# bab2min/Kiwi

Hardware: AMD Instinct MI355X
Metric: sentences/sec on batched analyze(), device kernels with inputs resident in HBM (dictionary scan + lattice + Viterbi/Knlm, top-1); host-to-host rate: see e2e (higher is better)
Workload: dtype int32+f32; 1 GPU; c2-64k: 65536 synthetic sentences ({'exact_jamo': 40}), synthetic 'full' model (kiwi_amd/synth.py), Knlm, top-1; sentences_per_gpu=65536, chunks_per_gpu=65536, jamo_per_gpu=2621440, parallelism=shard1, device_bytes=9402884427, rerun_chunks=0

## Files before the change

### include/kiwi_amd.h

```cpp
#ifndef KIWI_AMD_H
#define KIWI_AMD_H
#include <stddef.h>
#include <stdint.h>
#ifdef __cplusplus
extern "C" {
#endif

typedef struct kamd_engine* kamd_engine_h;
typedef struct kamd_batch* kamd_batch_h;
typedef struct kamd_results* kamd_results_h;

typedef struct
{
	uint32_t position, word_position, sent_position, line_number;
	uint16_t length; uint8_t tag; uint8_t sense_or_script;
	float score, typo_cost;
	uint32_t typo_form_id, paired_token, sub_sent_position;
	uint16_t dialect; uint16_t form_len;
	int32_t morph_id;
	uint64_t form_off;
} kamd_token_t;

kamd_engine_h kamd_open(const char* raw_model_path, int device);
kamd_engine_h kamd_open_dialects(const char* raw_model_path, int device, int enabled_dialects);
kamd_engine_h kamd_open_mode(const char* raw_model_path, int device, int lm_mode, int enabled_dialects);
void kamd_close(kamd_engine_h h);
const char* kamd_last_error(void);

int kamd_set_config(kamd_engine_h h, float cut_off_threshold, float space_penalty, float typo_cost_weight,
	uint32_t max_unk_form_size, uint32_t max_unk_form_size_followed_by_jclass, uint32_t space_tolerance, int integrate_allomorph);
int kamd_set_oov_chr_bias(kamd_engine_h h, float bias);
int kamd_set_oov_freq_params(kamd_engine_h h, float global_weight, float local_weight, float global_min_freq);

kamd_results_h kamd_analyze_batch(kamd_engine_h h, const uint16_t* texts, const uint64_t* offsets, uint32_t n,
	uint32_t top_n, uint64_t match_options, int open_ending, int host_threads);

kamd_batch_h kamd_stage(kamd_engine_h h, const uint16_t* texts, const uint64_t* offsets, uint32_t n, uint64_t match_options, int open_ending, int host_threads);
int kamd_run(kamd_engine_h h, kamd_batch_h b, float* ms_out);
kamd_results_h kamd_fetch(kamd_engine_h h, kamd_batch_h b, uint32_t top_n);
int kamd_batch_info(kamd_batch_h b, uint64_t* info3);
int kamd_batch_reruns(kamd_batch_h b, float* ms_out);
int kamd_batch_pool(kamd_batch_h b, uint64_t* out3);
void kamd_batch_close(kamd_batch_h b);

uint32_t kamd_res_texts(kamd_results_h r);
uint32_t kamd_res_size(kamd_results_h r, uint32_t text);
float kamd_res_prob(kamd_results_h r, uint32_t text, uint32_t index);
uint32_t kamd_res_token_num(kamd_results_h r, uint32_t text, uint32_t index);
const kamd_token_t* kamd_res_tokens(kamd_results_h r, uint32_t text, uint32_t index);
const uint16_t* kamd_res_forms(kamd_results_h r, uint32_t text);
uint64_t kamd_res_d2h_bytes(kamd_results_h r);
void kamd_res_close(kamd_results_h r);
size_t kamd_res_pack(kamd_results_h r, uint8_t* out, size_t cap);
kamd_results_h kamd_res_merge_strided(const uint8_t* const* parts, const size_t* sizes, uint32_t n_parts);

int kamd_debug_exact_math(const float* x, float* exp_out, float* log_out, uint32_t n);
int kamd_debug_exact_tanh(const float* x, float* tanh_out, uint32_t n);
int kamd_debug_cong_global(kamd_engine_h h, const uint32_t* ctx, const uint32_t* hist7, const uint32_t* next, const uint8_t* flags, float* out, uint32_t n);
uint64_t kamd_debug_match_pattern(uint16_t left, const uint16_t* text, uint32_t len, uint64_t match_options);
int kamd_debug_sbg_next(const char* raw_model_path, uint32_t* hist8, uint32_t* pos, uint32_t wid, float knlm_ll, float* ll_out);
typedef struct kamd_typo* kamd_typo_h;
kamd_typo_h kamd_typo_new(float continual_cost, float lengthening_cost);
void kamd_typo_close(kamd_typo_h t);
kamd_typo_h kamd_typo_default(int default_typo_set);
int kamd_typo_add(kamd_typo_h t, const uint16_t* orig, uint32_t n_orig, const uint16_t* error, uint32_t n_error, float cost, int left_cond, int dialect);
int kamd_typo_add_entry(kamd_typo_h t, const uint16_t* orig, uint32_t n_orig, const uint16_t* error, uint32_t n_error, float cost, int left_cond, int dialect);
int kamd_typo_set_costs(kamd_typo_h t, float continual_cost, float lengthening_cost);
int kamd_typo_scale(kamd_typo_h t, float scale);
int kamd_typo_prepare(kamd_typo_h t, int inverse);
size_t kamd_typo_graph(kamd_typo_h t, const uint16_t* text, uint32_t len, int allowed_dialect, int normalize_coda, uint8_t* out, size_t cap);
kamd_results_h kamd_analyze_batch_typo(kamd_engine_h h, kamd_typo_h t, float threshold, int allowed_dialect, const uint16_t* texts, const uint64_t* offsets, uint32_t n_texts,
                                       uint32_t top_n, uint64_t match_options, int open_ending, int host_threads);
kamd_batch_h kamd_stage_typo(kamd_engine_h h, kamd_typo_h t, float threshold, int allowed_dialect, const uint16_t* texts, const uint64_t* offsets, uint32_t n_texts,
                             uint64_t match_options, int open_ending, int host_threads);
typedef struct kamd_morphset* kamd_morphset_h;
kamd_morphset_h kamd_morphset_new(kamd_engine_h h);
int kamd_morphset_add(kamd_morphset_h m, const uint16_t* form, uint32_t len, int tag);
void kamd_morphset_close(kamd_morphset_h m);
kamd_results_h kamd_analyze_batch_opt(kamd_engine_h h, kamd_typo_h t, float threshold, int allowed_dialect, kamd_morphset_h blocklist,
                                      const uint16_t* texts, const uint64_t* offsets, uint32_t n_texts, uint32_t top_n, uint64_t match_options, int open_ending, int host_threads);
kamd_results_h kamd_analyze_batch_dialect(kamd_engine_h h, kamd_typo_h t, float threshold, int allowed_dialect, float dialect_cost, kamd_morphset_h blocklist,
                                          const uint16_t* texts, const uint64_t* offsets, uint32_t n_texts, uint32_t top_n, uint64_t match_options, int open_ending, int host_threads);
kamd_results_h kamd_analyze_pretokenized(kamd_engine_h h, const uint16_t* text, uint32_t len, uint32_t top_n, uint64_t match_options, int open_ending,
                                         const uint32_t* spans, uint32_t n_spans, const uint16_t* forms);
size_t kamd_typo_graph_device(kamd_engine_h h, kamd_typo_h t, const uint16_t* text, uint32_t len, int allowed_dialect, int normalize_coda, int use_device, uint8_t* out, size_t cap);
size_t kamd_typo_lattices(kamd_engine_h h, kamd_typo_h t, float threshold, int allowed_dialect, const uint16_t* text, uint32_t len, uint64_t match_options, uint8_t* out, size_t cap);
size_t kamd_dump_dict(kamd_engine_h h, uint8_t* out, size_t cap);
size_t kamd_dump_lattices(kamd_engine_h h, const uint16_t* text, uint32_t len, uint64_t match_options, uint8_t* out, size_t cap);

int kamd_cong_info(kamd_engine_h h, uint32_t* vocab, uint32_t* contexts, uint32_t* dim);
int kamd_cong_topk(kamd_engine_h h, int kind, const uint32_t* ids, const uint32_t* bg_ids, const float* weights, uint32_t n, uint32_t top_n,
                   uint32_t* out_ids, float* out_scores, uint32_t* out_counts);
int kamd_cong_pairs(kamd_engine_h h, int kind, const uint32_t* a, const uint32_t* b, uint32_t n, float* out);
int kamd_cong_to_context_id(kamd_engine_h h, const uint32_t* ids, uint32_t n, uint32_t* out_context);
int64_t kamd_cong_from_context_id(kamd_engine_h h, uint32_t context_id, uint32_t* out, uint64_t max_size);
int kamd_cong_inv_norms(kamd_engine_h h, int contexts, float* out);
int64_t kamd_cong_table(kamd_engine_h h, int contexts, uint8_t* out, uint64_t cap);

#ifdef __cplusplus
}
#endif
#endif
```

### kiwi_amd/csrc/capi_low.cpp

```cpp
#include <cstddef>
#include <cstring>
#include <memory>
#include <mutex>
#include <string>
#include "../../include/kiwi_amd.h"
#include "engine.hpp"
#include "sbg_eval.hpp"
#include "typo.hpp"

using namespace kamd;

struct kamd_engine { std::unique_ptr<Engine> e; };
struct kamd_batch { std::shared_ptr<StagedBatch> b; };
struct kamd_results { BatchResults r; };
static_assert(sizeof(kamd_token_t) == sizeof(FlatToken) && offsetof(kamd_token_t, form_off) == offsetof(FlatToken, formOff) && offsetof(kamd_token_t, morph_id) == offsetof(FlatToken, morph),
	"kamd_token_t is the layout of kamd::FlatToken");

namespace kamd { void exactMathProbe(const float* x, float* e, float* l, float* t, uint32_t n); }
namespace kamd { void conggProbe(const FlatModel& m, const uint32_t* ctx, const uint32_t* hist, const uint32_t* next, const uint8_t* flags, float* out, uint32_t n); }

namespace
{
	thread_local std::string lastError;
	template<class Fn, class R> R guarded(Fn&& fn, R fail)
	{
		try { return fn(); }
		catch (const std::exception& e) { lastError = e.what(); }
		catch (...) { lastError = "unknown error"; }
		return fail;
	}

	std::vector<std::pair<const char16_t*, size_t>> views(const uint16_t* texts, const uint64_t* offsets, uint32_t n)
	{
		std::vector<std::pair<const char16_t*, size_t>> v(n);
		for (uint32_t i = 0; i < n; ++i) v[i] = { (const char16_t*)texts + offsets[i], (size_t)(offsets[i + 1] - offsets[i]) };
		return v;
	}

	kamd_results* pack(BatchResults&& res) { return new kamd_results{ std::move(res) }; }

	const ResultSegment* ana(kamd_results_h r, uint32_t t, uint32_t i, uint32_t& a)
	{
		if (!r || t >= r->r.nTexts) return nullptr;
		size_t local;
		const ResultSegment& seg = r->r.locate(t, local);
		if (i >= seg.textAna[local + 1] - seg.textAna[local]) return nullptr;
		a = seg.textAna[local] + i;
		return &seg;
	}
}

extern "C"
{
	kamd_engine_h kamd_open(const char* path, int device)
	{
		return guarded([&]() { auto h = std::make_unique<kamd_engine>(); h->e.reset(new Engine(path, device)); return h.release(); }, (kamd_engine*)nullptr);
	}
	kamd_engine_h kamd_open_dialects(const char* path, int device, int enabled_dialects)
	{
		return guarded([&]() { auto h = std::make_unique<kamd_engine>(); h->e.reset(new Engine(path, device, Engine::LmMode::Auto, (uint32_t)enabled_dialects)); return h.release(); }, (kamd_engine*)nullptr);
	}
	kamd_engine_h kamd_open_mode(const char* path, int device, int lm_mode, int enabled_dialects)
	{
		return guarded([&]()
		{
			if (lm_mode < 0 || lm_mode > 4) throw std::invalid_argument{ "kamd_open_mode: lm_mode must be 0 .. 4" };
			static const Engine::LmMode modes[5] = { Engine::LmMode::Auto, Engine::LmMode::Knlm, Engine::LmMode::Sbg, Engine::LmMode::Cong, Engine::LmMode::CongGlobal };
			auto h = std::make_unique<kamd_engine>(); h->e.reset(new Engine(path, device, modes[lm_mode], (uint32_t)enabled_dialects)); return h.release();
		}, (kamd_engine*)nullptr);
	}
	void kamd_close(kamd_engine_h h) { delete h; }
// ... 155 lines not shown
				w.textAna = reinterpret_cast<const uint32_t*>(b + oTextAna); w.anaTok = reinterpret_cast<const uint32_t*>(b + oAnaTok); w.score = reinterpret_cast<const float*>(b + oScore);
				w.tok = reinterpret_cast<const FlatToken*>(b + oTok); w.forms = reinterpret_cast<const char16_t*>(b + oForms);
				bool ok = w.textAna[0] == 0 && w.textAna[w.nTexts] == w.nAna && w.anaTok[0] == 0 && w.anaTok[w.nAna] == nTok;
				for (uint32_t i = 0; ok && i < w.nTexts; ++i) ok = w.textAna[i] <= w.textAna[i + 1];
				for (uint32_t i = 0; ok && i < w.nAna; ++i) ok = w.anaTok[i] <= w.anaTok[i + 1];
				for (uint64_t i = 0; ok && i < nTok; ++i) ok = w.tok[i].formOff <= nForms && (uint64_t)w.tok[i].formLen + 1 <= nForms - w.tok[i].formOff;
				if (!ok) throw std::runtime_error{ "kamd_res_merge_strided: corrupt part (index tables out of range)" };
				total += w.nTexts;
			}
			for (uint32_t p = 0; p < n_parts; ++p) if (v[p].nTexts != (total + n_parts - 1 - p) / n_parts) throw std::runtime_error{ "kamd_res_merge_strided: parts are not an index-strided split" };
			auto res = std::make_unique<kamd_results>();
			BatchResults& R = res->r;
			R.nTexts = total;
			R.segs.resize((total + BatchResults::kSegTexts - 1) / BatchResults::kSegTexts);
			for (size_t g = 0; g < total; ++g)
			{
				const View& w = v[g % n_parts]; const size_t l = g / n_parts;
				ResultSegment& seg = R.segs[g / BatchResults::kSegTexts];
				for (uint32_t a = w.textAna[l]; a < w.textAna[l + 1]; ++a)
				{
					for (uint32_t i = w.anaTok[a]; i < w.anaTok[a + 1]; ++i)
					{
						FlatToken t = w.tok[i];
						const char16_t* fs = w.forms + t.formOff;
						t.formOff = seg.forms.size();
						seg.forms.insert(seg.forms.end(), fs, fs + t.formLen + 1);
						seg.toks.push_back(t);
					}
					seg.anaScore.push_back(w.score[a]);
					seg.anaTok.push_back((uint32_t)seg.toks.size());
				}
				seg.textAna.push_back((uint32_t)seg.anaScore.size());
			}
			return res.release();
		}, (kamd_results*)nullptr);
	}
	void kamd_res_close(kamd_results_h r) { delete r; }

	uint64_t kamd_debug_match_pattern(uint16_t left, const uint16_t* text, uint32_t len, uint64_t match_options)
	{
		const auto r = kamd::matchPattern((char16_t)left, (const char16_t*)text, (const char16_t*)text + len, match_options);
		return (uint64_t)r.first | ((uint64_t)r.second << 32);
	}

	int kamd_debug_exact_math(const float* x, float* exp_out, float* log_out, uint32_t n)
	{
		return guarded([&]() { kamd::exactMathProbe(x, exp_out, log_out, nullptr, n); return 0; }, -1);
	}
	int kamd_debug_exact_tanh(const float* x, float* tanh_out, uint32_t n)
	{
		return guarded([&]() { kamd::exactMathProbe(x, nullptr, nullptr, tanh_out, n); return 0; }, -1);
	}

	int kamd_debug_cong_global(kamd_engine_h h, const uint32_t* ctx, const uint32_t* hist7, const uint32_t* next, const uint8_t* flags, float* out, uint32_t n)
	{
		if (!h) return -1;
		return guarded([&]() { kamd::conggProbe(h->e->model(), ctx, hist7, next, flags, out, n); return 0; }, -1);
	}

	int kamd_debug_sbg_next(const char* raw_model_path, uint32_t* hist8, uint32_t* pos, uint32_t wid, float knlm_ll, float* ll_out)
	{
		return guarded([&]()
		{
			static std::mutex mu; static std::string cachedPath; static std::unique_ptr<FlatModel> cached;
			std::lock_guard<std::mutex> lk{ mu };
			if (!cached || cachedPath != raw_model_path) { cached.reset(new FlatModel); bakeModel(*cached, raw_model_path); cachedPath = raw_model_path; }
			const SbgView sv = cached->sbgView();
			if (!sv.present()) throw std::runtime_error{ "kamd_debug_sbg_next: the model has no SkipBigram tables" };
			uint32_t ring[8]; for (int i = 0; i < 8; ++i) ring[i] = hist8[i];
			uint32_t p = *pos & 7u;
			*ll_out = sbgNext(sv, ring, p, wid, knlm_ll);
			for (int i = 0; i < 8; ++i) hist8[i] = ring[i];
			*pos = p;
			return 0;
		}, -1);
	}

	struct kamd_typo { TypoTransformer tt; std::unique_ptr<PreparedTypo> prepared; };
	kamd_typo* kamd_typo_new(float continual_cost, float lengthening_cost)
	{
		return guarded([&]() { auto* t = new kamd_typo; t->tt.setContinualCost(continual_cost); t->tt.setLengtheningCost(lengthening_cost); return t; }, (kamd_typo*)nullptr);
	}
	void kamd_typo_close(kamd_typo* t) { delete t; }
	kamd_typo* kamd_typo_default(int set)
	{
		return guarded([&]() { auto* t = new kamd_typo; t->tt = defaultTypoSet(set); return t; }, (kamd_typo*)nullptr);
	}
	int kamd_typo_add(kamd_typo* t, const uint16_t* orig, uint32_t n_orig, const uint16_t* error, uint32_t n_error, float cost, int left_cond, int dialect)
	{
		if (!t) return -2;
		return guarded([&]() { t->tt.add(std::u16string{ (const char16_t*)orig, n_orig }, std::u16string{ (const char16_t*)error, n_error }, cost, (uint8_t)left_cond, (uint16_t)dialect); return 0; }, -1);
	}
	int kamd_typo_add_entry(kamd_typo* t, const uint16_t* orig, uint32_t n_orig, const uint16_t* error, uint32_t n_error, float cost, int left_cond, int dialect)
	{
		if (!t) return -2;
		return guarded([&]() { t->tt.addEntry(std::u16string{ (const char16_t*)orig, n_orig }, std::u16string{ (const char16_t*)error, n_error }, cost, (uint8_t)left_cond, (uint16_t)dialect); return 0; }, -1);
	}
	int kamd_typo_set_costs(kamd_typo* t, float continual_cost, float lengthening_cost)
	{
		if (!t) return -2;
		t->tt.setContinualCost(continual_cost); t->tt.setLengtheningCost(lengthening_cost);
		return 0;
	}
	int kamd_typo_scale(kamd_typo* t, float scale)
	{
		if (!t) return -2;
// ... 186 lines not shown
```

### kiwi_amd/csrc/engine.hip

```cpp
#include <hip/hip_runtime.h>
#include <unistd.h>
#include <cstdio>
#include <cstring>
#include <ctime>
#include <algorithm>
#include <atomic>
#include <cstdlib>
#include <chrono>
#include <condition_variable>
#include <functional>
#include <map>
#include <mutex>
#include <numeric>
#include <stdexcept>
#include <thread>
#include "engine.hpp"
#include "pretok.hpp"
#include "hostpool.hpp"
#include "post_fast.hpp"
#include "viterbi_kernel.hpp"
#include "exact_math.hpp"
#include "cong_global.hpp"
#include "chr_freq.hpp"
#include "typo_lattice_kernel.hpp"
#include "typo_graph_kernel.hpp"
#include "cong_query_kernel.hpp"

namespace kamd
{
	__global__ void k_dict_scan(ModelView M, BatchView B, WorkView W, uint32_t chunkBegin, uint32_t chunkCount);
	template<int GW> __global__ void k_build_lattice(ModelView M, BatchView B, WorkView W, SearchParams P, const uint32_t* chunkList, uint32_t chunkCount, uint32_t ldsBytes);
	__global__ void k_build_lattice_big(ModelView M, BatchView B, WorkView W, SearchParams P, uint32_t chunkBegin, uint32_t chunkCount, uint32_t ldsBytes, uint32_t waveLayout);
	__global__ void k_lattice_wave(ModelView M, BatchView B, WorkView W, SearchParams P, const uint32_t* chunkList, uint32_t chunkCount, uint32_t ldsBytes, uint32_t matchRatio16, uint32_t expandMode);
	__global__ void k_expand_cands(ModelView M, BatchView B, WorkView W, uint32_t chunkBegin, uint32_t chunkCount, uint32_t transposedOrder, const uint8_t* distMask);
	__global__ void k_expand_pos(ModelView M, BatchView B, WorkView W, SearchParams P, uint32_t chunkBegin, uint32_t chunkCount, const float* nodeTypoAll, uint32_t useChr);
	__global__ void k_unk_chr(ModelView M, BatchView B, WorkView W, ChrView C, uint32_t chunkBegin, uint32_t chunkCount, uint32_t hiTok, uint32_t loTok);
	__global__ void k_unk_chr_freq(ModelView M, BatchView B, WorkView W, ChrView C, ChrFreqParams Q, float chrBias, uint32_t chunkBegin, uint32_t chunkCount, uint32_t hiTok, uint32_t loTok);

	namespace
	{
		void hipCheck(hipError_t e, const char* what)
		{
			if (e != hipSuccess) throw std::runtime_error{ std::string{ "HIP error in " } + what + ": " + hipGetErrorString(e) };
		}
#define HIPCHECK(x) hipCheck((x), #x)

		struct DevBlockCache
		{
			struct Block { void* p; size_t cap; int device; };
			std::mutex mu; std::vector<Block> blocks; size_t bytes = 0;
			static constexpr size_t kMaxBlocks = 256, kMaxBytes = 64ull << 30;
			static void release(const Block& b) { if (b.device < 0) (void)hipHostFree(b.p); else (void)hipFree(b.p); }
			void* take(size_t n, size_t& capOut, int device)
			{
				std::lock_guard<std::mutex> g{ mu };
				size_t best = blocks.size();
				for (size_t i = 0; i < blocks.size(); ++i)
					if (blocks[i].device == device && blocks[i].cap >= n && blocks[i].cap <= 2 * n + (1u << 20) && (best == blocks.size() || blocks[i].cap < blocks[best].cap)) best = i;
				if (best == blocks.size()) return nullptr;
				void* p = blocks[best].p; capOut = blocks[best].cap; bytes -= capOut;
				blocks.erase(blocks.begin() + best);
				return p;
			}
			void give(void* p, size_t cap, int device)
			{
				{
					std::lock_guard<std::mutex> g{ mu };
					if (blocks.size() < kMaxBlocks && bytes + cap <= kMaxBytes) { blocks.push_back(Block{ p, cap, device }); bytes += cap; return; }
				}
				release(Block{ p, cap, device });
			}
			void trim()
			{
				std::lock_guard<std::mutex> g{ mu };
				for (auto& b : blocks) release(b);
				blocks.clear(); bytes = 0;
			}
		};
		DevBlockCache& devCache() { static DevBlockCache* c = new DevBlockCache; return *c; }
		int currentDevice() { int d = 0; (void)hipGetDevice(&d); return d; }

		struct DevBuf
		{
			void* p = nullptr; size_t cap = 0; int device = 0;
			DevBuf() = default;
			DevBuf(const DevBuf&) = delete;
			DevBuf& operator=(const DevBuf&) = delete;
// ... 100 lines not shown
		PinBuf hIn; DevBuf dIn;
		DevBuf dFullMask, dZAt, dNsToPos, dPosToNs, dCflag, dMask, dMoff, dNNs, dMatchForm, dNodes, dTmpNodes, dEndPosMap, dTmpIdx, dNNodes, dWideList, dExpanded;
		struct LatClass { uint32_t i, j, need, stream; };
		std::vector<std::vector<LatClass>> latClasses; std::vector<uint32_t> latSkip; uint32_t latClassesKey = 0xFFFFFFFFu;
		DevBuf dHist;
		uint32_t slotCap = 0; uint64_t ownStates = 0;
		DevBuf dStateAt, dSlotTable; uint64_t poolStates = 0, poolUsed = 0;
		TypoOption typo;
		TypoGraphDev typoDev;
		DevBuf dTypoGraph, dTypoLast, dTypoPool, dTypoChunks, dTypoTmp, dTypoMap, dTypoNs, dTypoPs, dTypoStates, dTypoSIdx, dTypoScratch, dNodeTypo, dTypoOrder, dBlockBits, dUnkChr, dUnkChrForm;
		TypoLatView tv{};
		DevBuf dPacks, dStates, dNodeStOff, dNodeStCnt, dReach, dTokens, dResults, dOrder;
		DevBuf dPosRecs, dPosDesc, dPosPrev, dPosNodeRec, dPosMask;
		DevBuf dOutPaths, dOutTokens, dOutCounters; uint32_t outPathCap = 0, outTokCap = 0;
		PinBuf hOut, hOut2;
		uint64_t outBytes = 0;
		BatchView bv{}; WorkView wv{};
		const DevChunkResult* hResults = nullptr; const DevPathHeader* hPaths = nullptr; const DevToken* hTokens = nullptr; size_t hTokCount = 0;
		bool ran = false;
		hipEvent_t evDone = nullptr; bool launched = false; uint32_t launchS = 1;
		~StagedBatch()
		{
			if (evDone) (void)hipEventDestroy(evDone);
			if (prepBlocks.size() >= 64)
			{
				try { HostPool::instance().run(prepBlocks.size(), 16, hostThreads, [&](size_t i0, size_t i1, int) { for (size_t i = i0; i < i1; ++i) { PrepBlock dead = std::move(prepBlocks[i]); } }); }
				catch (...) {}
			}
		}
		uint32_t subBatches = 0;
		uint32_t topN = 1;
		std::vector<size_t> overIdx; std::vector<std::vector<PathResult>> overPaths; uint32_t rerunChunks = 0; float rerunMs = 0;
		std::vector<uint32_t> typoNeed, typoOrder;
		std::vector<uint32_t> order;
	};

	struct Engine::Impl
	{
		std::shared_ptr<FlatModel> modelOwner;
		FlatModel& model;
		explicit Impl(std::shared_ptr<FlatModel> m) : modelOwner(std::move(m)), model(*modelOwner) {}
		ModelView dview{};
		std::vector<std::unique_ptr<DevBuf>> modelBufs;
		hipStream_t stream = nullptr, stream2 = nullptr;
		hipStream_t latStream[3] = { nullptr, nullptr, nullptr };
		hipStream_t streamCopy = nullptr;
		hipEvent_t lastDone = nullptr, joinEv = nullptr; bool haveLast = false;
		hipEvent_t latFork = nullptr, latJoin[3] = { nullptr, nullptr, nullptr };
		std::vector<hipEvent_t> evs;
		int subBatches = 0;
		int device = 0;
		uint32_t persistBlocks = 0;
		int latticeGroupForced = 0;
		bool latticeWave = true;
		uint32_t latticeRatio16 = kLatticeWideRatio16; bool latticeRatioForced = false;
		uint32_t stateScale64[2] = { 0, 0 }; bool stateScaleForced = false;
		uint32_t poolFrac64 = 64; bool poolForced = false;
		uint32_t latticeLdsBudget = 64 * 1024;
		uint32_t latticeWaveBudget = 128 * 1024;
		bool groupLanesForced = false; int wpsForced = 0;
		bool posPath = true;
		bool wantCongGlobal = false;
		bool posPathForced = false;
		bool posPathTypo = true;
		int posGroupForced = 0;
		int groupLanes = 16;
		DevBuf bigScratch, counter, posScratch;
		uint32_t posContSlots = 256;
		ChrView chr{};
		CongDev cong{}; bool hasCong = false;
		CongGDev congG{}; bool hasCongG = false;
		bool histStates() const { return hasSbg || hasCongG; }
		uint32_t histBlocksPerCu() const { static const int v = std::getenv("KAMD_HIST_BLOCKS") ? std::atoi(std::getenv("KAMD_HIST_BLOCKS")) : 12; return (uint32_t)std::min(16, std::max(1, v)); }
		uint32_t histSlots() const { return persistBlocks / 12 * histBlocksPerCu() * ((groupLanesForced && groupLanes == 16) ? 4u : 1u); }
		SbgDev sbg{}; bool hasSbg = false; DevBuf sbgScratch;
		std::recursive_mutex deviceMu;
		TokenTemplates tokTmpl;
		std::mutex congMu; hipStream_t congStream = nullptr; bool congNormsOnDevice = false;
		DevBuf congIds, congBg, congW, congScores, congOutIds, congOutScores, congInvOut, congInvCtx;
		std::once_flag congNormOnce, congMapOnce;
		std::vector<float> congNormOut, congNormCtx;
		std::vector<std::vector<uint32_t>> congWordMap;

		static constexpr size_t kTempForms = 4096, kTempMorphs = 8192, kTempChars = 1u << 17, kTempCand = 16384, kTempChunks = 16384;
		template<class T> const T* up(const std::vector<T>& v, size_t slack = 0)
		{
			modelBufs.emplace_back(new DevBuf);
			DevBuf& b = *modelBufs.back();
			b.ensure(std::max<size_t>((v.size() + slack) * sizeof(T), 16));
			if (!v.empty()) HIPCHECK(hipMemcpy(b.p, v.data(), v.size() * sizeof(T), hipMemcpyHostToDevice));
			return b.as<T>();
		}
	};

	int Engine::deviceIndex() const { return impl->device; }
	void Engine::bindThread() const { (void)hipSetDevice(impl->device); }
	int Engine::visibleDevices()
	{
		int n = 0;
		if (hipGetDeviceCount(&n) != hipSuccess) return 0;
		return n;
	}

	Engine::Engine(const std::string& path, int device, LmMode lm, uint32_t enabledDialects) : impl(new Impl(std::make_shared<FlatModel>()))
	{
		bakeModel(impl->model, path, enabledDialects);
// ... 28 lines not shown
		for (auto& ls : impl->latStream) HIPCHECK(hipStreamCreateWithFlags(&ls, hipStreamNonBlocking));
		{
			int least = 0, greatest = 0;
			const bool plain = [] { const char* e = std::getenv("KAMD_COPY_PRIORITY"); return !(e && std::atoi(e) == 1); }();
			if (plain || hipDeviceGetStreamPriorityRange(&least, &greatest) != hipSuccess || least == greatest) HIPCHECK(hipStreamCreateWithFlags(&impl->streamCopy, hipStreamNonBlocking));
			else HIPCHECK(hipStreamCreateWithPriority(&impl->streamCopy, hipStreamNonBlocking, greatest));
		}
		HIPCHECK(hipEventCreateWithFlags(&impl->lastDone, hipEventDisableTiming)); HIPCHECK(hipEventCreateWithFlags(&impl->joinEv, hipEventDisableTiming));
		HIPCHECK(hipEventCreate(&impl->latFork)); for (auto& ev : impl->latJoin) HIPCHECK(hipEventCreate(&ev));

		if (const char* sb = std::getenv("KAMD_SUBBATCHES")) impl->subBatches = std::atoi(sb);
		const FlatModel& m = impl->model;
		ModelView& v = impl->dview;
		v.h = m.h;
		using I_ = Engine::Impl;
		v.forms = impl->up(m.forms, I_::kTempForms); v.formChars = impl->up(m.formChars, I_::kTempChars); v.formCand = impl->up(m.formCand, I_::kTempCand);
		{
			std::vector<MorphRec> dm = m.morphs;
			for (size_t i = 0; i < dm.size(); ++i) { dm[i].feat = (uint16_t)m.morphPath[i]; dm[i].prevFlags = (uint8_t)(m.morphPath[i] >> 16); }
			v.morphs = impl->up(dm, I_::kTempMorphs);
			std::vector<CandStatic> unk(2);
			for (int k = 0; k < 2; ++k)
			{
				const uint32_t mid = (k == 0 ? T_NNG : T_NNP) + 1u;
				std::memcpy(&unk[k].m0, &dm[mid], 32);
				const uint32_t firstWid = (dm[mid].flags & MF_SINGLE) ? dm[mid].lmId : m.chunkLm[dm[mid].chunkOff];
				unk[k].x = Quad{ mid, firstWid, 0, 0 };
			}
			v.unkPacks = impl->up(unk);
		}
		v.chunkMorph = impl->up(m.chunkMorph, I_::kTempChunks); v.chunkLm = impl->up(m.chunkLm, I_::kTempChunks); v.chunkPos = impl->up(m.chunkPos, 2 * I_::kTempChunks);
		v.sbInfo = impl->up(m.sbInfo, I_::kTempMorphs); v.morphPath = impl->up(m.morphPath, I_::kTempMorphs);
		v.trie = impl->up(m.trie); v.trieKeys = impl->up(m.trieKeys); v.trieChild = impl->up(m.trieChild); v.trieRoot = impl->up(m.trieRoot);
		v.trieEdges = impl->up(m.trieEdges); v.trieEdgeMask = m.trieEdgeMask;
		v.lmNodes = impl->up(m.lmNodes); v.lmKeys = impl->up(m.lmKeys); v.lmValues = impl->up(m.lmValues); v.lmRoot = impl->up(m.lmRoot);
		if (m.congDim)
		{
			v.lmHash = impl->up(m.congHash); v.lmHashMask = m.congHashMask; v.lmRoot2 = impl->up(m.congRoot2); v.lmBackoff = impl->up(m.congBackoff);
			v.h.bosNode = 0;
			impl->cong = CongDev{ impl->up(m.congCtxEmb), impl->up(m.congOutEmb), m.congDim, m.congDim + 8, m.congVlTMax, m.congVlBits };
			impl->hasCong = true;
			if (impl->wantCongGlobal)
			{
				if (!m.congWindow) throw std::runtime_error{ "Cannot open ConG model with distant tokens: the file has no window sections" };
				if (m.congWindow != 7) throw std::runtime_error{ "kiwi_amd: CoNgram window size must be 7 (the reference instantiates CoNgramState<7> only)" };
				CongGDev& g = impl->congG;
				g.ctxConf = impl->up(m.congCtxConf); g.distEmb = impl->up(m.congDistEmb); g.distConf = impl->up(m.congDistConf); g.posConf = impl->up(m.congPosConf);
				g.distMask = impl->up(m.congDistMask); g.window = m.congWindow; g.keyBytes = m.congKeyBytes; g.hist = nullptr; g.itemScratch = nullptr;
				impl->hasCongG = true;
			}
		}
		else { v.lmHash = impl->up(m.lmHash); v.lmHashMask = m.lmHashMask; v.lmRoot2 = impl->up(m.lmRoot2); v.lmBackoff = impl->up(m.lmBackoff); }
		v.lmHtxNode = (m.congDim || m.lmHtxNode.empty()) ? nullptr : impl->up(m.lmHtxNode);
		v.formDialect = nullptr;
		v.morphDialect = m.morphDialect.empty() ? nullptr : impl->up(m.morphDialect, I_::kTempMorphs);
		if (v.morphDialect) HIPCHECK(hipMemset(const_cast<uint16_t*>(v.morphDialect) + m.morphDialect.size(), 0, 2 * I_::kTempMorphs));
		v.formUnkChr = nullptr; v.formChrTok = nullptr;
		v.lmChain = nullptr;
		if (!m.congDim && !m.lmBackoff.empty())
		{
			std::vector<uint32_t> chain(2 * m.lmBackoff.size());
			for (size_t n = 0; n < m.lmBackoff.size(); ++n)
			{
				const uint32_t l1 = n ? (uint32_t)((int64_t)n + m.lmBackoff[n].lower) : 0u;
				const uint32_t l2 = l1 ? (uint32_t)((int64_t)l1 + m.lmBackoff[l1].lower) : 0u;
				chain[2 * n] = l1; chain[2 * n + 1] = l2;
			}
			v.lmChain = impl->up(chain);
		}
		if (m.chrDim)
		{
			ChrView c = m.chrView();
			c.ctxEmb = impl->up(m.chrCtxEmb); c.outEmb = impl->up(m.chrOutEmb); c.nodes = impl->up(m.chrNodes); c.keys = impl->up(m.chrKeys); c.values = impl->up(m.chrValues);
			c.root = impl->up(m.chrRoot); c.inv = m.chrInv.empty() ? nullptr : impl->up(m.chrInv);
			c.depth = impl->up(m.chrDepth); c.freqTab = impl->up(m.chrFreqTab);
			impl->chr = c;
			v.formUnkChr = impl->up(m.formUnkChr, I_::kTempForms); v.formChrTok = impl->up(m.formChrTok, I_::kTempChars);
		}
		if (!m.sbgPtrs.empty())
		{
			const SbgView sv = m.sbgView();
			SbgDev& d = impl->sbg;
			d.ptrs = impl->up(m.sbgPtrs); d.keys = impl->up(m.sbgKeys); d.comps = impl->up(m.sbgComps); d.discnts = impl->up(m.sbgDiscnts); d.valid = impl->up(m.sbgValid);
			d.vocabSize = sv.vocabSize; d.logWindowSize = sv.logWindowSize; d.hist = nullptr; d.itemScratch = nullptr;
			impl->hasSbg = true;
		}
		hipDeviceProp_t prop;
		HIPCHECK(hipGetDeviceProperties(&prop, device));
		impl->persistBlocks = (uint32_t)prop.multiProcessorCount * 12;
		if (const char* g = std::getenv("KAMD_GROUP_LANES"))
		{
			const int v = std::atoi(g);
			if (v == 4 || v == 8 || v == 16 || v == 32 || v == 64) { impl->groupLanes = v; impl->groupLanesForced = true; }
			else throw std::runtime_error{ "KAMD_GROUP_LANES must be 4, 8, 16, 32 or 64" };
		}
		if (const char* w = std::getenv("KAMD_WPS")) { const int v = std::atoi(w); if (v == 2 || v == 3) impl->wpsForced = v; else throw std::runtime_error{ "KAMD_WPS must be 2 or 3" }; }
		if (const char* pp = std::getenv("KAMD_POS_PATH")) { impl->posPath = std::atoi(pp) != 0; impl->posPathForced = std::atoi(pp) == 2; impl->posPathTypo = std::atoi(pp) != 3; }
		if (const char* pg = std::getenv("KAMD_POS_G")) { const int v = std::atoi(pg); if (v == 8 || v == 16) impl->posGroupForced = v; else throw std::runtime_error{ "KAMD_POS_G must be 8 or 16" }; }
		if (const char* pc = std::getenv("KAMD_POS_CONT")) impl->posContSlots = (uint32_t)std::max(0, std::min(4096, std::atoi(pc)));
		if (const char* lg = std::getenv("KAMD_LATTICE_GROUP")) { const int v = std::atoi(lg); if (v == 16 || v == 64) impl->latticeGroupForced = v; }
		if (const char* lw = std::getenv("KAMD_LATTICE_WAVE")) impl->latticeWave = std::atoi(lw) != 0;
		if (const char* ss = std::getenv("KAMD_STATE_SCALE")) { impl->stateScale64[0] = impl->stateScale64[1] = (uint32_t)std::min(64, std::max(1, std::atoi(ss))); impl->stateScaleForced = true; }
		if (const char* ps = std::getenv("KAMD_STATE_POOL")) { impl->poolFrac64 = (uint32_t)std::min(4096, std::max(0, std::atoi(ps))); impl->poolForced = true; }
		if (const char* lr = std::getenv("KAMD_LATTICE_RATIO")) { impl->latticeRatio16 = (uint32_t)std::min(4096, std::max(4, std::atoi(lr))); impl->latticeRatioForced = true; }
		if (const char* l = std::getenv("KAMD_LATTICE_LDS")) { impl->latticeLdsBudget = (uint32_t)std::min(64 * 1024, std::max(0, std::atoi(l))); impl->latticeWaveBudget = (uint32_t)std::min(128 * 1024, std::max(0, std::atoi(l))); }
		if (impl->latticeWaveBudget > 64 * 1024) HIPCHECK(hipFuncSetAttribute(reinterpret_cast<const void*>(&k_lattice_wave), hipFuncAttributeMaxDynamicSharedMemorySize, (int)impl->latticeWaveBudget));
		impl->counter.ensure(256);
	}

	Engine::~Engine()
	{
		if (impl)
		{
			(void)hipSetDevice(impl->device);
			(void)hipDeviceSynchronize();
			for (auto& e : impl->evs) if (e) (void)hipEventDestroy(e);
			impl->modelBufs.clear();
			impl->bigScratch.release(); impl->posScratch.release(); impl->counter.release(); impl->sbgScratch.release();
			for (DevBuf* d : { &impl->congIds, &impl->congBg, &impl->congW, &impl->congScores, &impl->congOutIds, &impl->congOutScores, &impl->congInvOut, &impl->congInvCtx }) d->release();
			devCache().trim();
			if (impl->stream) (void)hipStreamDestroy(impl->stream);
			if (impl->stream2) (void)hipStreamDestroy(impl->stream2);
			if (impl->congStream) (void)hipStreamDestroy(impl->congStream);
			for (auto ls : impl->latStream) if (ls) (void)hipStreamDestroy(ls);
			if (impl->streamCopy) (void)hipStreamDestroy(impl->streamCopy);
			if (impl->lastDone) (void)hipEventDestroy(impl->lastDone);
			if (impl->joinEv) (void)hipEventDestroy(impl->joinEv);
			if (impl->latFork) (void)hipEventDestroy(impl->latFork);
			for (auto ev : impl->latJoin) if (ev) (void)hipEventDestroy(ev);
		}
	}

	const FlatModel& Engine::model() const { return impl->model; }
	bool Engine::usesCong() const { return impl->hasCong; }
	bool Engine::usesSbg() const { return impl->hasSbg; }
	bool Engine::usesCongGlobal() const { return impl->hasCongG; }
	uint32_t Engine::congWindow() const { return impl->hasCong ? impl->model.congWindow : 0u; }

	namespace
	{
		struct HostTimer
		{
			bool on = std::getenv("KAMD_HOST_TIMING") != nullptr; const char* what; std::chrono::steady_clock::time_point t0 = std::chrono::steady_clock::now();
			double cpu0 = on ? cpuNow() : 0.0;
			explicit HostTimer(const char* w) : what(w) {}
			static double cpuNow() { timespec ts; clock_gettime(CLOCK_PROCESS_CPUTIME_ID, &ts); return ts.tv_sec * 1e3 + ts.tv_nsec * 1e-6; }
			void lap(const char* name)
			{
				if (!on) return;
				const auto t1 = std::chrono::steady_clock::now(); const double c1 = cpuNow();
				fprintf(stderr, "[host] %s: %s %.2f ms (process CPU %.1f ms)\n", what, name, std::chrono::duration<double, std::milli>(t1 - t0).count(), c1 - cpu0);
				t0 = t1; cpu0 = c1;
			}
		};
// ... 298 lines not shown
				t.stateOff = (uint32_t)stateTop; t.stateCap = (uint32_t)std::min<uint64_t>(((uint64_t)t.graphCnt * 16 + 64) * sc, 0x7FFFFFFF); stateTop += t.stateCap;
				gch[c].graphOff = t.graphOff; gch[c].graphCap = t.graphCnt; gch[c].scrOff = (uint32_t)scrTop; gch[c].scrCap = T.scratchCapFor(t.nChars, t.graphCnt);
				scrTop += gch[c].scrCap;
				if (mapTop > 0xFFFFFFF0ull || stateTop > 0xFFFFFFF0ull || graphTop > 0xFFFFFFF0ull || scrTop > 0xFFFFFFF0ull) throw std::runtime_error{ "batch too large for 32-bit typo scratch offsets: split the batch" };
			}
			b.typoNeed.resize(nC); for (size_t c = 0; c < nC; ++c) b.typoNeed[c] = tch[c].ldsNeed;
			const size_t graphSize = std::max<uint64_t>(graphTop, 1);
			b.dTypoGraph.ensure(graphSize * sizeof(TypoGraphNode) + 64); b.dTypoLast.ensure(graphSize * 2 + 64);
			dTemp.ensure(graphSize * sizeof(TypoGraphNode) + 64);
			dMatches.ensure(scrTop * 8 + 16); dBp.ensure(scrTop * 4 + 16); dEpm.ensure(scrTop * 8 + 16); dRev.ensure(scrTop * 4 + 16); dCnt.ensure(scrTop * 4 + 16);
			upload(dGch, gch, s);
			gv.chunks = dGch.as<TypoGraphChunk>(); gv.matches = dMatches.as<uint2>(); gv.bp = dBp.as<uint32_t>(); gv.epm = dEpm.as<uint2>(); gv.rev = dRev.as<uint32_t>(); gv.cnt = dCnt.as<uint32_t>();
			gv.graph = b.dTypoGraph.as<TypoGraphNode>(); gv.graphLast = b.dTypoLast.as<uint8_t>(); gv.temp = dTemp.as<TypoGraphNode>();
			launchTypoGraph(gd.tables, gv, (uint32_t)nC, false, s);
			HIPCHECK(hipGetLastError());
			upload(b.dTypoChunks, tch, s);
			b.dTypoTmp.ensure(totNodes * sizeof(TypoLatNode) + 64); b.dTypoMap.ensure(mapTop * 8 + 64); b.dTypoNs.ensure(nsTop * 2 + 64); b.dTypoPs.ensure(nsTop * 2 + 64);
			b.dTypoStates.ensure(stateTop * sizeof(TypoState) + 64); b.dTypoSIdx.ensure(graphSize * 8 + 64); b.dTypoScratch.ensure(totNodes * 12 + 64);
			b.dNodeTypo.ensure(totNodes * 4 + 64);
			TypoLatView& v = b.tv;
			v = TypoLatView{};
			v.chars = bv.chars; v.cls = bv.cls; v.script = bv.script; v.patterns = bv.patterns;
			v.graph = b.dTypoGraph.as<TypoGraphNode>(); v.graphLast = b.dTypoLast.as<uint8_t>(); v.pool = gd.tables.pool; v.chunks = b.dTypoChunks.as<TypoLatChunk>();
			v.nodes = b.dTypoTmp.as<TypoLatNode>(); v.nodesFinal = nullptr; v.endPosMap = b.dTypoMap.as<uint2>(); v.nsToPos = b.dTypoNs.as<uint16_t>(); v.posToNs = b.dTypoPs.as<uint16_t>();
			v.states = b.dTypoStates.as<TypoState>(); v.stateIdx = b.dTypoSIdx.as<uint32_t>(); v.scratch = b.dTypoScratch.as<uint32_t>();
			v.devNodes = w.nodes; v.nodeTypo = b.dNodeTypo.as<float>(); v.nNodes = w.nNodes; v.results = w.results;
			HIPCHECK(hipStreamSynchronize(s));
		}
		HIPCHECK(hipStreamSynchronize(s));
		tmL.lap("waiting for the upload");
		b.ran = false;
	}

	__global__ void k_exact_math_probe(const float* x, float* e, float* l, float* t, uint32_t n)
	{
		const uint32_t i = blockIdx.x * blockDim.x + threadIdx.x;
		if (i >= n) return;
		if (e) e[i] = exact::expf_glibc(x[i]);
		if (l) l[i] = exact::logf_glibc(x[i]);
		if (t) t[i] = exact::tanhf_glibc(x[i]);
	}
	void exactMathProbe(const float* x, float* e, float* l, float* t, uint32_t n)
	{
		DevBuf dx, de, dl, dt;
		dx.ensure((size_t)n * 4 + 16); de.ensure((size_t)n * 4 + 16); dl.ensure((size_t)n * 4 + 16); dt.ensure((size_t)n * 4 + 16);
		HIPCHECK(hipMemcpy(dx.p, x, (size_t)n * 4, hipMemcpyHostToDevice));
		hipLaunchKernelGGL(k_exact_math_probe, dim3((n + 255) / 256), dim3(256), 0, 0, dx.as<float>(), e ? de.as<float>() : (float*)nullptr, l ? dl.as<float>() : (float*)nullptr, t ? dt.as<float>() : (float*)nullptr, n);
		HIPCHECK(hipGetLastError());
		if (e) HIPCHECK(hipMemcpy(e, de.p, (size_t)n * 4, hipMemcpyDeviceToHost));
		if (l) HIPCHECK(hipMemcpy(l, dl.p, (size_t)n * 4, hipMemcpyDeviceToHost));
		if (t) HIPCHECK(hipMemcpy(t, dt.p, (size_t)n * 4, hipMemcpyDeviceToHost));
	}

	__global__ void k_congg_probe(CongView C, const uint32_t* ctx, const uint32_t* hist, const uint32_t* next, const uint8_t* flags, float* out, uint32_t n)
	{
		const uint32_t i = blockIdx.x * blockDim.x + threadIdx.x;
		if (i >= n) return;
		uint32_t h[7];
		for (int k = 0; k < 7; ++k) h[k] = hist[7ull * i + k];
		const bool matrix = flags[i] & 1, outFirst = flags[i] & 2;
		if (C.distant(next[i])) out[i] = matrix ? congg::scoreMatrix(C, ctx[i], h, next[i], outFirst) : congg::scoreSingle(C, ctx[i], h, next[i]);
		else out[i] = outFirst ? congScoreOutputFirst(C, ctx[i], next[i]) : congScore(C, ctx[i], next[i]);
	}
	void conggProbe(const FlatModel& m, const uint32_t* ctx, const uint32_t* hist, const uint32_t* next, const uint8_t* flags, float* out, uint32_t n)
	{
		if (!m.congDim || !m.congWindow) throw std::runtime_error{ "the model has no CoNgram window sections" };
		DevBuf dCtxEmb, dOutEmb, dDistEmb, dCtxConf, dDistConf, dPosConf, dMask, dCtx, dHist, dNext, dFlags, dOut;
		auto up = [](DevBuf& b, const void* p, size_t bytes) { b.ensure(bytes + 16); HIPCHECK(hipMemcpy(b.p, p, bytes, hipMemcpyHostToDevice)); };
		up(dCtxEmb, m.congCtxEmb.data(), m.congCtxEmb.size()); up(dOutEmb, m.congOutEmb.data(), m.congOutEmb.size()); up(dDistEmb, m.congDistEmb.data(), m.congDistEmb.size());
		up(dCtxConf, m.congCtxConf.data(), m.congCtxConf.size() * 4); up(dDistConf, m.congDistConf.data(), m.congDistConf.size() * 4);
		up(dPosConf, m.congPosConf.data(), m.congPosConf.size() * 4); up(dMask, m.congDistMask.data(), m.congDistMask.size());
		up(dCtx, ctx, (size_t)n * 4); up(dHist, hist, (size_t)n * 28); up(dNext, next, (size_t)n * 4); up(dFlags, flags, n);
		dOut.ensure((size_t)n * 4 + 16);
		CongView C;
		C.dim = m.congDim; C.stride = m.congDim + 8; C.nCtx = m.congCtx; C.vocabSize = m.congVocab; C.window = m.congWindow; C.keyBytes = m.congKeyBytes;
		C.ctxEmb = dCtxEmb.as<uint8_t>(); C.outEmb = dOutEmb.as<uint8_t>(); C.distEmb = dDistEmb.as<uint8_t>();
		C.ctxConf = dCtxConf.as<float>(); C.distConf = dDistConf.as<float>(); C.posConf = dPosConf.as<float>(); C.distMask = dMask.as<uint8_t>();
		hipLaunchKernelGGL(k_congg_probe, dim3((n + 63) / 64), dim3(64), 0, 0, C, dCtx.as<uint32_t>(), dHist.as<uint32_t>(), dNext.as<uint32_t>(), dFlags.as<uint8_t>(), dOut.as<float>(), n);
		HIPCHECK(hipGetLastError());
		HIPCHECK(hipMemcpy(out, dOut.p, (size_t)n * 4, hipMemcpyDeviceToHost));
	}

	static SearchParams makeParams(const EngineConfig& c, uint64_t match, uint32_t topN = 1, const TypoOption* opt = nullptr)
	{
		SearchParams p{};
		p.allowedDialect = opt ? opt->allowedDialect : 0u; p.dialectCost = opt ? opt->dialectCost : 3.f;
		p.match = match; p.cutOff = c.cutOffThreshold; p.spacePenalty = c.spacePenalty; p.typoCostWeight = c.typoCostWeight;
		p.oovRuleScale = c.oovRuleScale; p.oovRuleBias = c.oovRuleBias;
		p.oovGlobalWeight = c.oovGlobalWeight; p.oovLocalWeight = c.oovLocalWeight; p.oovGlobalMinFreq = c.oovGlobalMinFreq; p.oovChrFreqBias = c.oovChrBias;
		p.oovChrBias = ((match >> 8) & 3) > 1 ? 0.f : c.oovChrBias;
		p.maxUnk = c.maxUnkFormSize; p.maxUnkJ = c.maxUnkFormSizeFollowedByJClass; p.spaceTol = c.spaceTolerance;
		p.splitComplex = (match & M_SPLIT_COMPLEX) ? 1 : 0; p.splitSaisiot = (match & M_SPLIT_SAISIOT) ? 1 : 0; p.mergeSaisiot = (match & M_MERGE_SAISIOT) ? 1 : 0;
		p.topN = topN;
		p.smallMax = 128; p.mediumMax = 512; p.bucketCap = 128;
		if (const char* l = std::getenv("KAMD_CONTAINER_LIMITS"))
		{
			unsigned a = 0, b = 0, c = 0;
			if (std::sscanf(l, "%u,%u,%u", &a, &b, &c) == 3 && a <= b && c >= 1) { p.smallMax = a; p.mediumMax = b; p.bucketCap = c; }
			else throw std::runtime_error{ "KAMD_CONTAINER_LIMITS must be small,medium,bucket" };
		}
		return p;
	}

#ifdef KAMD_TIMELINE
	static void* gTimeline = nullptr;
#endif
// ... 108 lines not shown
					while (i < c1 && needOf(b.order[i]) > budget) ++i;
					while (i < c1)
					{
						const uint32_t need = needOf(b.order[i]);
						uint32_t j = i + 1;
						while (j < c1 && (uint64_t)needOf(b.order[j]) * 4 >= (uint64_t)need * 3) ++j;
						b.latClasses[k].push_back({ i, j, need, 0u });
						i = j;
					}
					std::vector<size_t> byCost(b.latClasses[k].size());
					std::iota(byCost.begin(), byCost.end(), (size_t)0);
					auto cost = [&](size_t t) { const auto& c = b.latClasses[k][t]; return (uint64_t)(c.j - c.i) * c.need; };
					std::stable_sort(byCost.begin(), byCost.end(), [&](size_t x, size_t y) { return cost(x) > cost(y); });
					uint64_t load[4] = { 0, 0, 0, 0 };
					for (size_t t : byCost) { const uint32_t st = (uint32_t)(std::min_element(load, load + 4) - load); b.latClasses[k][t].stream = st; load[st] += cost(t); }
				}
				b.latClassesKey = classesKey;
			}
		}
		tm.lap("work order, size classes, scratch");
		for (uint32_t k = 0; k < S; ++k)
		{
			const uint32_t c0 = (uint32_t)((uint64_t)nC * k / S), c1 = (uint32_t)((uint64_t)nC * (k + 1) / S), cn = c1 - c0;
			hipEvent_t* e = &I.evs[6 * (size_t)k];
			HIPCHECK(hipEventRecord(e[0], sA));
			if (b.typo.typo)
			{
				TypoLatView tv = b.tv;
				tv.lengtheningCost = b.typo.typo->lengtheningCost();
				tv.threshold = b.typo.threshold; tv.maxUnk = sp.maxUnk; tv.maxUnkJ = sp.maxUnkJ; tv.spaceTol = sp.spaceTol; tv.match = sp.match;
				HIPCHECK(hipEventRecord(e[1], sA));
				{
					uint32_t i = c0;
					while (i < c1 && b.typoNeed[b.typoOrder[i]] > I.latticeLdsBudget) ++i;
					while (i < c1)
					{
						const uint32_t need = b.typoNeed[b.typoOrder[i]];
						uint32_t j = i + 1;
						while (j < c1 && (uint64_t)b.typoNeed[b.typoOrder[j]] * 4 >= (uint64_t)need * 3) ++j;
						launchTypoLatticeLds(I.dview, tv, b.dTypoOrder.as<uint32_t>() + i, j - i, need, sA);
						i = j;
					}
				}
				tv.chunks += c0;
				launchTypoLatticeRest(I.dview, tv, cn, I.latticeLdsBudget, sA);
			}
			else
			{
			hipLaunchKernelGGL(k_dict_scan, dim3((cn + 3) / 4), dim3(256), 0, sA, I.dview, b.bv, b.wv, c0, cn);
			HIPCHECK(hipEventRecord(e[1], sA));
			{
				const bool wave = I.latticeWave && I.latticeGroupForced == 0;
				const uint32_t ratio16 = I.latticeRatio16 | (getenv("KAMD_LATTICE_STATS") ? 0x4000u : 0u);
				static const bool fuseExpand = !(getenv("KAMD_LATTICE_EXPAND") && std::atoi(getenv("KAMD_LATTICE_EXPAND")) == 0);
				const bool posEarly = b.wv.posRecs && sp.topN == 1 && !I.groupLanesForced && S <= 8 && (!b.typo.typo || I.posPathTypo);
				const uint32_t expandMode = (fuseExpand && posEarly && !b.wv.unkChr && !b.wv.blockBits) ? (1u | (I.hasCong ? 2u : 0u)) : 0u;
				if (getenv("KAMD_LATTICE_PROFILE")) { lwProf.ensure((size_t)nC * 64); HIPCHECK(hipMemsetAsync(lwProf.p, 0, (size_t)nC * 64, sA)); b.wv.beacon = lwProf.as<uint32_t>(); }
				const uint32_t budget = b.pretok ? 0u : wave ? I.latticeWaveBudget : I.latticeLdsBudget;
				uint32_t nClass = 0;
				if (wave && k) HIPCHECK(hipMemsetAsync(b.dOutCounters.as<uint32_t>() + 3, 0, 4, sA));
				if (wave) { HIPCHECK(hipEventRecord(I.latFork, sA)); for (auto ls : I.latStream) HIPCHECK(hipStreamWaitEvent(ls, I.latFork, 0)); }
				for (const auto& lc : b.latClasses[k])
				{
					const uint32_t i = lc.i, j = lc.j, need = lc.need;
					static const uint32_t dbgStop = std::getenv("KAMD_LATTICE_STOP") ? (uint32_t)std::atoi(std::getenv("KAMD_LATTICE_STOP")) : 0u;
					const uint32_t need16 = (need + 15u) & ~15u;
					const bool four = I.latticeGroupForced == 16 && need16 * 4 <= 64 * 1024;
					hipStream_t sL = (wave && lc.stream) ? I.latStream[lc.stream - 1] : sA;
					++nClass;
					if (wave) hipLaunchKernelGGL(k_lattice_wave, dim3(j - i), dim3(64), need, sL, I.dview, b.bv, b.wv, sp, b.dOrder.as<uint32_t>() + i, j - i, need | (dbgStop << 24), ratio16, expandMode);
					else if (four) hipLaunchKernelGGL(k_build_lattice<16>, dim3((j - i + 3) / 4), dim3(64), need16 * 4, sA, I.dview, b.bv, b.wv, sp, b.dOrder.as<uint32_t>() + i, j - i, need16 | (dbgStop << 24));
					else hipLaunchKernelGGL(k_build_lattice<64>, dim3(j - i), dim3(64), need, sA, I.dview, b.bv, b.wv, sp, b.dOrder.as<uint32_t>() + i, j - i, need | (dbgStop << 24));
				}
				if (wave) for (int t = 0; t < 3; ++t) { HIPCHECK(hipEventRecord(I.latJoin[t], I.latStream[t])); HIPCHECK(hipStreamWaitEvent(sA, I.latJoin[t], 0)); }
				if (wave && budget) hipLaunchKernelGGL(k_lattice_wave, dim3(std::min(cn, 16384u)), dim3(64), budget, sA, I.dview, b.bv, b.wv, sp, b.dOrder.as<uint32_t>() + c0, std::min(cn, 16384u), budget, kLatticeWideRatio16 | kLatticeWideBit | (ratio16 & 0x4000u), expandMode);
				hipLaunchKernelGGL(k_build_lattice_big, dim3((cn + 63) / 64), dim3(64), 0, sA, I.dview, b.bv, b.wv, sp, c0, cn, budget, wave ? (ratio16 & 0x3FFFu) : 0u);
			}
			}
			hipLaunchKernelGGL(k_expand_cands, dim3(cn), dim3(64), 0, sA, I.dview, b.bv, b.wv, c0, cn, I.hasCong ? 1u : 0u, I.hasCongG ? I.congG.distMask : (const uint8_t*)nullptr);
			if (b.wv.unkChrForm)
				hipLaunchKernelGGL(k_unk_chr_freq, dim3(cn), dim3(64), 0, sA, I.dview, b.bv, b.wv, I.chr, ChrFreqParams{ sp.oovGlobalWeight, sp.oovLocalWeight, sp.oovGlobalMinFreq }, sp.oovChrFreqBias,
					c0, cn, chrToken(0xD800, identifySpecialChr(0xD800)), chrToken(0xDC00, identifySpecialChr(0xDC00)));
			else if (b.wv.unkChr)
				hipLaunchKernelGGL(k_unk_chr, dim3(cn), dim3(64), 0, sA, I.dview, b.bv, b.wv, I.chr, c0, cn, chrToken(0xD800, identifySpecialChr(0xD800)), chrToken(0xDC00, identifySpecialChr(0xDC00)));
			const bool usePos = b.wv.posRecs && sp.topN == 1 && !I.groupLanesForced && S <= 8 && (!b.typo.typo || I.posPathTypo);
			if (usePos)
				hipLaunchKernelGGL(k_expand_pos, dim3(cn), dim3(64), 0, sA, I.dview, b.bv, b.wv, sp, c0, cn, b.typo.typo ? b.dNodeTypo.as<float>() : (const float*)nullptr, ((I.hasCong && b.wv.unkChr) ? 1u : 0u) | (I.hasCong ? 2u : 0u));
			HIPCHECK(hipEventRecord(e[2], sA));
			HIPCHECK(hipStreamWaitEvent(sB, e[2], 0));
			HIPCHECK(hipEventRecord(e[3], sB));
			const uint32_t blocks = std::min(I.persistBlocks, (cn + nGroups - 1) / nGroups);
			WorkView wv = b.wv;
			wv.beacon = nullptr;
			wv.posHandOver = usePos ? I.counter.as<uint32_t>() + 48 + k : nullptr;
			if (usePos && I.posContSlots)
			{
				I.posScratch.ensure((size_t)I.posContSlots * groupScratchBytes * std::min(S, 2u));
				wv.posScratch = I.posScratch.as<uint8_t>() + (size_t)(k & 1) * ((S > 1) ? (size_t)I.posContSlots * groupScratchBytes : 0);
				wv.posContCounter = I.counter.as<uint32_t>() + 56 + (k & 7); wv.posContSlots = I.posContSlots;
			}
#ifdef KAMD_TIMELINE
			static DevBuf tlBuf;
			tlBuf.ensure((size_t)nC * 128);
			HIPCHECK(hipMemsetAsync(tlBuf.p, 0, (size_t)nC * 128, sB));
			wv.beacon = tlBuf.as<uint32_t>(); gTimeline = tlBuf.p;
#endif
#ifndef KAMD_TIMELINE
// ... 145 lines not shown
								fprintf(stderr, "\n");
							}
						}
						fprintf(stderr, "[hangdump] pos beacon stages:"); for (int l = 0; l < 16; ++l) fprintf(stderr, " %d:%u", l, hist[l]); fprintf(stderr, "\n");
					}
					fflush(stderr);
					_exit(7);
				}
			}
		}
		HIPCHECK(hipGetLastError());
		HIPCHECK(hipEventRecord(I.joinEv, sA)); HIPCHECK(hipStreamWaitEvent(sB, I.joinEv, 0));
		if (!b.evDone) HIPCHECK(hipEventCreateWithFlags(&b.evDone, hipEventDisableTiming | hipEventBlockingSync));
		HIPCHECK(hipEventRecord(b.evDone, sB)); HIPCHECK(hipEventRecord(I.lastDone, sB));
		I.haveLast = true; b.launched = true; b.launchS = S;
		tm.lap("enqueueing the launches");
		if (!wait) return t;
		HIPCHECK(hipStreamSynchronize(sA));
		HIPCHECK(hipStreamSynchronize(sB));
		tm.lap("waiting for the kernels");
		afterLaunch(I, b, t, true);
		return t;
	}

	static void afterLaunch(Engine::Impl& I, StagedBatch& b, KernelTimes& t, bool timed)
	{
		const uint32_t nC = (uint32_t)b.refs.size();
		const uint32_t S = b.launchS;
		if (getenv("KAMD_POS_BEACON") && getenv("KAMD_POS_PHASES") && posBeacon.p)
		{
			std::vector<uint32_t> bc((size_t)nC * 64);
			HIPCHECK(hipMemcpy(bc.data(), posBeacon.p, bc.size() * 4, hipMemcpyDeviceToHost));
			double acc[14] = {}, steps = 0;
			for (uint32_t c = 0; c < nC; ++c) { for (int k2 = 0; k2 < 14; ++k2) acc[k2] += bc[(size_t)c * 64 + 16 + k2]; steps += bc[(size_t)c * 64 + 31]; }
			static const char* names[14] = { "loop/prefetch", "nodes+records", "round header+mapping", "record decode", "scoring after the LM step (rules, key)", "arg-max rotations", "emit", "end of rounds", "prune+counters", "retries+flags", "commit", "end stage", "wait for parent state + record", "LM step" };
			double tot = 0; for (int k2 = 0; k2 < 14; ++k2) tot += acc[k2];
			fprintf(stderr, "[pos phases] cycles per step (group-lane-0 clock; %0.f steps):", steps);
			for (int k2 = 0; k2 < 14; ++k2) fprintf(stderr, " %s %.0f (%.0f%%);", names[k2], steps ? acc[k2] / steps : 0.0, tot ? 100.0 * acc[k2] / tot : 0.0);
			fprintf(stderr, " total %.0f\n", steps ? tot / steps : 0.0);
		}
		if (I.latticeWave && !I.latticeRatioForced && !b.typo.typo && nC >= 256 && b.capScale == 1 && !b.isRerun)
		{
			uint32_t c16[16] = {};
			HIPCHECK(hipMemcpyAsync(c16, b.dOutCounters.p, 64, hipMemcpyDeviceToHost, I.streamCopy)); HIPCHECK(hipStreamSynchronize(I.streamCopy));
			uint32_t want = (c16[13] * 16u * 5u / 4u + 99u) / 100u + 2u;
			if (c16[4] + c16[5] > nC / 256) want = std::max(want, I.latticeRatio16 * 3u / 2u);
			want = std::max(want, I.latticeRatio16 - std::min(I.latticeRatio16, (I.latticeRatio16 + 7u) / 8u));
			I.latticeRatio16 = std::min(kLatticeWideRatio16, std::max(12u, want));
		}
		if (getenv("KAMD_LATTICE_PROFILE") && lwProf.p)
		{
			std::vector<uint32_t> rec((size_t)nC * 16);
			HIPCHECK(hipMemcpy(rec.data(), lwProf.p, rec.size() * 4, hipMemcpyDeviceToHost));
			double pr[13] = {}; uint32_t seen = 0;
			for (uint32_t c = 0; c < nC; ++c) { if (!rec[(size_t)c * 16]) continue; ++seen; for (int k2 = 0; k2 < 13; ++k2) pr[k2] += rec[(size_t)c * 16 + k2]; }
			static const char* names[13] = { "stage", "type pass", "match ops", "groups", "clear", "by-time", "by-start", "publish", "checks", "ranks", "sweep+prefix", "emit", "pack offsets" };
			double tot = 0; for (int k2 = 0; k2 < 13; ++k2) tot += pr[k2];
			fprintf(stderr, "[lattice profile] clock ticks per wavefront (%u chunks):", seen);
			for (int k2 = 0; k2 < 13; ++k2) fprintf(stderr, " %s %.0f (%.0f%%);", names[k2], seen ? pr[k2] / seen : 0.0, tot ? 100.0 * pr[k2] / tot : 0.0);
			fprintf(stderr, " total %.0f\n", seen ? tot / seen : 0.0);
		}
		if (getenv("KAMD_LATTICE_STATS"))
		{
			uint32_t c16[16] = {};
			HIPCHECK(hipMemcpy(c16, b.dOutCounters.p, 64, hipMemcpyDeviceToHost));
			std::vector<uint8_t> ex(nC); std::vector<PosDesc> pd;
			HIPCHECK(hipMemcpy(ex.data(), b.dExpanded.p, nC, hipMemcpyDeviceToHost));
			uint32_t nEx = 0, nProg = 0;
			for (uint32_t c = 0; c < nC; ++c) if (ex[c]) { ++nEx; if (b.wv.posDesc) { PosDesc d; HIPCHECK(hipMemcpy(&d, b.wv.posDesc + b.nodeBase[c], sizeof(d), hipMemcpyDeviceToHost)); nProg += d.firstRec != 0; } }
			fprintf(stderr, "[lattice wave] records written by the lattice kernel: %u chunks (%u with a position program)\n", nEx, nProg);
			fprintf(stderr, "[lattice wave] chunks %u: built %u (%.2f rounds each); handed over: matches %u, ops %u, long span / rounds %u, no end node %u, long node %u, no start %u; ops per text unit: mean %.2f, max %.2f (matches: max %.2f)\n",
				(uint32_t)nC, c16[10], c16[10] ? (double)c16[11] / c16[10] : 0.0, c16[4], c16[5], c16[6], c16[7], c16[8], c16[9], c16[15] ? (double)c16[14] / c16[15] : 0.0, c16[12] / 100.0, c16[13] / 100.0);
		}
		if (b.wv.posRecs && getenv("KAMD_POS_STATS"))
		{
			std::vector<DevChunkResult> res(nC); std::vector<uint32_t> nn(nC);
			HIPCHECK(hipMemcpy(res.data(), b.dResults.p, nC * sizeof(DevChunkResult), hipMemcpyDeviceToHost));
			HIPCHECK(hipMemcpy(nn.data(), b.dNNodes.p, nC * 4, hipMemcpyDeviceToHost));
			double frac = 0; uint32_t early = 0, carried = 0, atStart = 0, seen = 0, why[16] = {};
			for (uint32_t c = 0; c < nC; ++c)
			{
				const uint32_t at = res[c].pad & 0xFFFFFFu;
				if (!at || !nn[c]) continue;
				++seen;
				if (at == kPosChunkDone && (res[c].pad >> 24)) { ++carried; ++why[(res[c].pad >> 24) & 15]; if (carried <= 8) fprintf(stderr, "[pos] carried on: chunk %u of %u, reason %u\n", c, (uint32_t)nC, (res[c].pad >> 24) & 15); continue; }
				if (at == kPosChunkDone || at + 1 >= nn[c]) continue;
				++early; frac += (double)at / nn[c]; atStart += at <= 1; ++why[(res[c].pad >> 24) & 15];
			}
			{ uint32_t c32[32]; HIPCHECK(hipMemcpy(c32, b.dOutCounters.p, 128, hipMemcpyDeviceToHost)); fprintf(stderr, "[pos] positions left to the general search by k_expand_pos: more than 16 nodes %u, more than 16 records %u, no record %u, node-level (feeds its step / nothing to evaluate / > 256 predecessors) %u\n", c32[20], c32[21], c32[22], c32[23]); }
			fprintf(stderr, "[pos] chunks %u (searched %u), carried on in the general search by the kernel itself %u, left to k_best_path %u (%.2f %%), of those from the start %u, mean hand-over point %.2f of the lattice; reasons: static %u, ring %u, container %u, record size %u, staging %u, retry %u, disconnected %u, no program %u, test cannot run %u\n",
				nC, seen, carried, early, seen ? 100.0 * early / seen : 0.0, atStart, early ? frac / early : 0.0, why[1], why[2], why[3], why[4], why[5], why[6], why[7], why[8], why[9]);
		}
#ifdef KAMD_TIMELINE
		if (getenv("KAMD_TIMELINE_PRINT") && gTimeline)
		{
			std::vector<unsigned long long> tl((size_t)nC * 16);
			HIPCHECK(hipMemcpy(tl.data(), gTimeline, tl.size() * 8, hipMemcpyDeviceToHost));
			unsigned long long t0 = ~0ull, tEnd = 0;
			for (uint32_t c = 0; c < nC; ++c) if (tl[16ull * c]) { t0 = std::min(t0, tl[16ull * c]); tEnd = std::max(tEnd, tl[16ull * c + 2]); }
			std::vector<double> start, nodes, fin, perNode;
			for (uint32_t c = 0; c < nC; ++c)
			{
				if (!tl[16ull * c] || !tl[16ull * c + 2]) continue;
				start.push_back((tl[16ull * c] - t0) * 0.01); nodes.push_back((tl[16ull * c + 1] - tl[16ull * c]) * 0.01); fin.push_back((tl[16ull * c + 2] - tl[16ull * c + 1]) * 0.01);
				perNode.push_back(nodes.back() / std::max<double>(1.0, (double)(uint32_t)tl[16ull * c + 3]));
			}
			auto stat = [](std::vector<double> v, const char* name)
			{
				if (v.empty()) return;
				std::sort(v.begin(), v.end());
				double sum = 0; for (double x : v) sum += x;
				fprintf(stderr, "[timeline] %-26s mean %9.1f  p50 %9.1f  p90 %9.1f  p99 %9.1f  max %9.1f  (us, n=%zu)\n", name, sum / v.size(), v[v.size() / 2], v[v.size() * 9 / 10], v[v.size() * 99 / 100], v.back(), v.size());
			};
			fprintf(stderr, "[timeline] first chunk start -> last chunk end: %.1f us\n", (tEnd - t0) * 0.01);
			static const char* phName[12] = { "ph0 node setup", "ph1 cand record + misc", "ph2 scoring (+Knlm)", "ph3 emission: write states", "ph4 prune", "ph5 bookkeeping", "ph6 passes/reach", "ph7 scoring: before the LM step", "ph8 classify (pack load)", "ph9 batch formation + key table build", "ph10 scoring: Knlm step", "ph11" };
			for (int k = 0; k < 10; ++k)
			{
				std::vector<double> v;
				for (uint32_t c = 0; c < nC; ++c) if (tl[16ull * c] && tl[16ull * c + 2]) v.push_back(tl[16ull * c + 4 + k] * 0.01 / std::max<double>(1.0, (double)(uint32_t)tl[16ull * c + 3]));
				stat(v, phName[k]);
			}
			{
				std::vector<double> mhz;
				for (uint32_t c = 0; c < nC; ++c) if (tl[16ull * c] && tl[16ull * c + 1] > tl[16ull * c]) mhz.push_back((double)tl[16ull * c + 15] / ((tl[16ull * c + 1] - tl[16ull * c]) * 0.01));
				stat(mhz, "shader clock (MHz)");
// ... 1101 lines not shown
```

### kiwi_amd/csrc/flat_model.hpp

```cpp
#pragma once
#include <cstdint>
#include <cmath>
#include <string>
#include <vector>
#include "kchars.hpp"

namespace kamd
{
	enum FormFlag : uint8_t
	{
		FF_ZCODA_APPENDABLE = 1, FF_ZSIOT_APPENDABLE = 2, FF_HAS_JCLASS = 4, FF_HAS_ANY_FULL = 8,
		FF_FIRST_IS_CODA = 16,
		FF_IS_STAG = 32,
		FF_STARTS_WITH_A = 64,
		FF_ENDS_WITH_SSC = 128,
	};
	struct FormRec
	{
		uint32_t candOff;
		uint32_t charOff;
		uint16_t candCnt;
		uint8_t len;
		uint8_t numSpaces;
		uint8_t flags;
// ... 53 lines not shown
	constexpr int32_t TRIE_NONE = -1, TRIE_SUBMATCH = -2;
	constexpr uint16_t LF_STR_SSC = 1u << 13, LF_PREV_ZSIOT = 1u << 14, LF_TAG_SSC = 1u << 15;

	struct LmSlot { uint32_t node, wid; int32_t value; float ll; };
	static_assert(sizeof(LmSlot) == 16, "LmSlot");
	constexpr uint32_t LM_SLOT_EMPTY = 0xFFFFFFFFu;
	struct LmRootRec { int32_t value; float ll; };
	struct LmBackoff { int32_t lower; float gamma; };
	KAMD_HD uint32_t lmHashOf(uint32_t node, uint32_t wid) { uint32_t h = node * 0x9E3779B1u ^ (wid * 0x85EBCA77u); h ^= h >> 15; h *= 0x2C1B3C6Du; h ^= h >> 13; return h; }

	struct LmNodeRec
	{
		uint32_t nextOff, numNexts;
		int32_t lower;
		float ll, gamma;
	};
	static_assert(sizeof(LmNodeRec) == 20, "LmNodeRec");

	struct ModelHeader
	{
		uint32_t nForms, nMorphs, vocabSize, nTrieNodes, nTrieEdges, nLmNodes, nLmEdges;
		int32_t bosNode;
		float unkLl;
		uint32_t specialMorph[6];
		uint32_t maxFormLen;
		uint32_t lmOrder;
		uint32_t lmKeyBytes;
	};

	struct ModelView
	{
		ModelHeader h;
		const FormRec* forms;
		const uint16_t* formChars;
		const uint32_t* formCand;
		const MorphRec* morphs;
		const uint32_t* chunkMorph;
		const uint32_t* chunkLm;
		const uint8_t* chunkPos;
		const uint8_t* sbInfo;
		const uint32_t* morphPath;
		const TrieNodeRec* trie;
		const uint16_t* trieKeys;
		const uint32_t* trieChild;
		const uint32_t* trieRoot;
		const LmNodeRec* lmNodes;
		const uint32_t* lmKeys;
		const int32_t* lmValues;
		const int32_t* lmRoot;
		const LmSlot* lmHash; uint32_t lmHashMask;
		const LmRootRec* lmRoot2;
		const LmBackoff* lmBackoff;
		const void* unkPacks;
		const int32_t* lmHtxNode;
		const float* formUnkChr;
		const uint16_t* formChrTok;
		const uint16_t* formDialect; const uint16_t* morphDialect;
		const uint32_t* lmChain;
		const TrieEdgeSlot* trieEdges; uint32_t trieEdgeMask;
	};

	struct SbgView
	{
		uint32_t vocabSize = 0, windowSize = 0;
		const uint32_t* ptrs = nullptr;
		const uint32_t* keys = nullptr;
		const float* comps = nullptr;
		const float* discnts = nullptr;
		const uint8_t* valid = nullptr;
		float logWindowSize = 0;
		bool present() const { return vocabSize != 0; }
	};

	struct CongNodeRec { uint32_t nextOff, numNexts; int32_t lower; uint32_t value; };
	struct CongView
	{
		uint32_t dim = 0, stride = 0, nCtx = 0, vocabSize = 0;
		const uint8_t* ctxEmb = nullptr; const uint8_t* outEmb = nullptr;
		const CongNodeRec* nodes = nullptr; const uint32_t* keys = nullptr; const int32_t* values = nullptr; const int32_t* root = nullptr;
		uint32_t rootSize = 0;
		uint32_t vlTMax = 0xFFFFFFFFu, vlBits = 0;
		uint32_t window = 0;
		uint32_t keyBytes = 4;
		const float* ctxConf = nullptr;
		const uint8_t* distEmb = nullptr;
		const float* distConf = nullptr;
		const float* posConf = nullptr;
		const uint8_t* distMask = nullptr;
		bool present() const { return dim != 0; }
		KAMD_HD bool distant(uint32_t w) const { return window && (distMask[w >> 3] >> (w & 7) & 1); }
	};
	KAMD_HD float congScore(const CongView& C, uint32_t c, uint32_t w)
	{
		const int8_t* a = reinterpret_cast<const int8_t*>(C.ctxEmb + (size_t)c * C.stride);
		const int8_t* b = reinterpret_cast<const int8_t*>(C.outEmb + (size_t)w * C.stride);
		int32_t acc = 0;
		for (uint32_t k = 0; k < C.dim; ++k) acc += (int32_t)a[k] * (int32_t)b[k];
		float cs, os, bias;
		__builtin_memcpy(&cs, a + C.dim, 4); __builtin_memcpy(&bias, a + C.dim + 4, 4); __builtin_memcpy(&os, b + C.dim, 4);
		return (float)acc * cs * os + bias;
	}

	KAMD_HD float congCosine(int32_t dot, float scaleQ, float scaleI, float invNormQ, float invNormI)
	{
		const float s = (float)dot * scaleQ * scaleI;
		return s * (invNormQ * invNormI);
// ... 161 lines not shown
		std::vector<float> congCtxConf, congDistConf, congPosConf; std::vector<uint8_t> congDistEmb, congDistMask; uint32_t congWindow = 0, congKeyBytes = 4;
		bool congGlobal = false;

		CongView congView() const
		{
			CongView v;
			if (!congDim) return v;
			v.dim = congDim; v.stride = congDim + 8; v.nCtx = congCtx; v.vocabSize = congVocab; v.rootSize = (uint32_t)congRoot.size(); v.vlTMax = congVlTMax; v.vlBits = congVlBits;
			v.ctxEmb = congCtxEmb.data(); v.outEmb = congOutEmb.data();
			v.nodes = congNodes.data(); v.keys = congKeys.data(); v.values = congValues.data(); v.root = congRoot.data();
			v.keyBytes = congKeyBytes;
			if (congGlobal && congWindow)
			{
				v.window = congWindow; v.ctxConf = congCtxConf.data(); v.distEmb = congDistEmb.data(); v.distConf = congDistConf.data();
				v.posConf = congPosConf.data(); v.distMask = congDistMask.data();
			}
			return v;
		}

		ChrView chrView() const
		{
			ChrView v;
			if (!chrDim) return v;
			v.dim = chrDim; v.stride = chrDim + 8; v.nCtx = chrCtx; v.vocab = chrVocab;
			v.ctxEmb = chrCtxEmb.data(); v.outEmb = chrOutEmb.data(); v.nodes = chrNodes.data(); v.keys = chrKeys.data(); v.values = chrValues.data(); v.root = chrRoot.data();
			v.inv = chrInv.empty() ? nullptr : chrInv.data(); v.bosNode = chrBosNode; v.bosCtx = chrBosCtx;
			v.depth = chrDepth.empty() ? nullptr : chrDepth.data(); v.freqTab = chrFreqTab.empty() ? nullptr : chrFreqTab.data(); v.bosCtxPacked = chrBosCtxPacked; v.hasFreq = chrHasFreq;
			return v;
		}

		SbgView sbgView() const
		{
			SbgView v;
			if (sbgPtrs.empty()) return v;
			v.vocabSize = (uint32_t)sbgDiscnts.size(); v.windowSize = sbgWindow;
			v.ptrs = sbgPtrs.data(); v.keys = sbgKeys.data(); v.comps = sbgComps.data(); v.discnts = sbgDiscnts.data(); v.valid = sbgValid.data();
			v.logWindowSize = std::log((float)sbgWindow);
			return v;
		}

		ModelView view() const
		{
			ModelView v;
			v.h = h;
			v.forms = forms.data(); v.formChars = formChars.data(); v.formCand = formCand.data();
			v.morphs = morphs.data(); v.chunkMorph = chunkMorph.data(); v.chunkLm = chunkLm.data(); v.chunkPos = chunkPos.data();
			v.sbInfo = sbInfo.data(); v.morphPath = morphPath.data();
			v.trie = trie.data(); v.trieKeys = trieKeys.data(); v.trieChild = trieChild.data(); v.trieRoot = trieRoot.data();
			v.lmNodes = lmNodes.data(); v.lmKeys = lmKeys.data(); v.lmValues = lmValues.data(); v.lmRoot = lmRoot.data();
			v.lmHash = lmHash.data(); v.lmHashMask = lmHashMask; v.lmRoot2 = lmRoot2.data(); v.lmBackoff = lmBackoff.data();
			v.lmHtxNode = lmHtxNode.empty() ? nullptr : lmHtxNode.data();
			v.formUnkChr = formUnkChr.empty() ? nullptr : formUnkChr.data();
			v.formChrTok = formChrTok.empty() ? nullptr : formChrTok.data();
			v.lmChain = nullptr;
			v.trieEdges = trieEdges.empty() ? nullptr : trieEdges.data(); v.trieEdgeMask = trieEdgeMask;
			v.formDialect = formDialect.empty() ? nullptr : formDialect.data(); v.morphDialect = morphDialect.empty() ? nullptr : morphDialect.data();
			return v;
		}

		std::u16string formStr(uint32_t f) const
		{
			return std::u16string{ (const char16_t*)formChars.data() + forms[f].charOff, forms[f].len };
		}
	};

	void bakeModel(FlatModel& out, const std::string& rawModelPath, uint32_t enabledDialects = 0);
	void buildTrieEdges(FlatModel& m);
	struct TempEntries
	{
		struct Form { std::u16string str; std::vector<uint32_t> cands; };
		struct Chunk { uint32_t morph; uint8_t begin, end; };
		struct Morph { uint32_t tempForm; uint8_t tag; uint32_t lmId; std::vector<Chunk> chunks; };
		std::vector<Form> forms; std::vector<Morph> morphs;
	};
	void bakeModelWithTemps(FlatModel& out, const std::string& rawModelPath, uint32_t enabledDialects, const TempEntries& temps);
	struct TempOverlay
	{
		uint32_t nBaseForms = 0, nBaseMorphs = 0;
		std::vector<FormRec> forms;
		std::vector<uint16_t> formChars;
		std::vector<uint32_t> formCand;
		std::vector<MorphRec> morphs;
		std::vector<uint32_t> chunkMorph, chunkLm; std::vector<uint8_t> chunkPos;
		std::vector<uint8_t> sbInfo; std::vector<uint32_t> morphPath, morphKform;
		std::vector<float> formUnkChr; std::vector<uint16_t> formChrTok;
		bool empty() const { return forms.empty(); }
	};
	void bakeTempsOverlay(const FlatModel& base, const TempEntries& temps, TempOverlay& out);
	std::vector<uint8_t> dumpDict(const FlatModel& m);
	std::vector<uint32_t> findMorphemes(const FlatModel& m, const char16_t* s, size_t n, uint8_t tag);
	int32_t formIdOfString(const FlatModel& m, const std::u16string& nrm);
	std::vector<uint32_t> blockBitsOf(const FlatModel& m, const std::vector<uint32_t>& ids);
	float chrScoreHost(const ChrView& C, const uint16_t* s, size_t n);
}
```

### kiwi_amd/csrc/lattice_kernels.hip

```cpp
#include <hip/hip_runtime.h>
#include "device_types.hpp"
#include "feature.hpp"
#include "lattice_connect.hpp"
#include "lattice_expand.hpp"
#include "chr_freq.hpp"

namespace kamd
{
	__device__ __forceinline__ uint32_t trieChild(const ModelView& M, uint32_t node, uint16_t c, int32_t& value)
	{
		if (node == 0) { const uint32_t ch = M.trieRoot[c]; value = ch ? M.trie[ch].value : TRIE_NONE; return ch; }
		uint32_t h = trieEdgeHash(node, c) & M.trieEdgeMask;
		for (;;)
		{
			const uint4 s = reinterpret_cast<const uint4*>(M.trieEdges)[h];
			if (s.x == node && s.y == (uint32_t)c) { value = (int32_t)s.w; return s.z; }
			if (s.x == TRIE_EDGE_EMPTY) { value = TRIE_NONE; return 0; }
			h = (h + 1) & M.trieEdgeMask;
		}
	}

	__global__ void __launch_bounds__(256) k_dict_scan(ModelView M, BatchView B, WorkView W, uint32_t chunkBegin, uint32_t chunkCount)
	{
		const uint32_t lane = threadIdx.x & 63;
// ... 728 lines not shown
		W.nNodes[chunk] = nConn;
		if (nConn <= 2) W.results[chunk].status = CS_NO_LATTICE;
	}

	__global__ void __launch_bounds__(64) k_expand_cands(ModelView M, BatchView B, WorkView W, uint32_t chunkBegin, uint32_t chunkCount, uint32_t transposedOrder, const uint8_t* distMask)
	{
		if (blockIdx.x >= chunkCount) return;
		const uint32_t chunk = chunkBegin + blockIdx.x;
		if (W.results[chunk].status != CS_OK || W.expanded[chunk]) return;
		const uint32_t nBase = W.nodeBase[chunk], G = W.nNodes[chunk];
		CandStatic* packs = W.packs + W.packBase[chunk];
		const uint32_t* blk = W.blockBits;
		auto blocked = [&](uint32_t m2) -> bool { return blk && ((blk[m2 >> 5] >> (m2 & 31)) & 1); };
		for (uint32_t i = 1 + threadIdx.x; i + 1 < G; i += blockDim.x)
		{
			const DevNode nd = W.nodes[nBase + i];
			if (nd.form == NOFORM) continue;
			const uint32_t candOff = M.forms[nd.form].candOff;
			uint32_t kept = 0;
			for (uint32_t k = 0; k < nd.candCnt; ++k)
			{
				const uint32_t mid = M.formCand[candOff + k];
				if (blocked(mid)) continue;
				++kept;
				const CandStatic o = candStaticOf(M, mid);
				uint32_t at = 0;
				if (transposedOrder)
				{
					auto cls = [&](uint32_t m2) -> uint32_t
					{
						const MorphRec r = M.morphs[m2];
						uint32_t c2 = 2u * candClassOf(r.tag, r.socket, r.flags);
						if (distMask && c2 == 4u) { const uint32_t fw = (r.flags & MF_SINGLE) ? r.lmId : M.chunkLm[r.chunkOff]; c2 += (distMask[fw >> 3] >> (fw & 7)) & 1u; }
						return c2;
					};
					const uint32_t mine = cls(mid);
					for (uint32_t j = 0; j < nd.candCnt; ++j)
					{
						if (j == k) continue;
						const uint32_t mj = M.formCand[candOff + j];
						if (blocked(mj)) continue;
						const uint32_t other = cls(mj);
						if (other < mine || (other == mine && j < k)) ++at;
					}
				}
				else if (blk) { for (uint32_t j = 0; j < k; ++j) if (!blocked(M.formCand[candOff + j])) ++at; }
				else at = k;
				packs[nd.packOff + at] = o;
			}
			if (kept != nd.candCnt) W.nodes[nBase + i].candCnt = (uint16_t)kept;
		}
	}

	__global__ void __launch_bounds__(64) k_expand_pos(ModelView M, BatchView B, WorkView W, SearchParams P, uint32_t chunkBegin, uint32_t chunkCount, const float* nodeTypoAll, uint32_t useChr)
	{
		if (blockIdx.x >= chunkCount) return;
		const uint32_t lane = threadIdx.x;
		const uint32_t chunk = chunkBegin + blockIdx.x;
		if (W.expanded[chunk]) return;
		const uint32_t nBase = W.nodeBase[chunk];
		PosDesc* desc = W.posDesc + nBase;
		if (lane == 0) { desc[0].firstNode = 0; desc[0].nNodes = 0; desc[0].flags = 0; desc[0].firstRec = 0; desc[0].nRec = 0; }
		if (W.results[chunk].status != CS_OK) return;
		const uint32_t G = W.nNodes[chunk];
		const uint32_t nUniq = B.spOff[chunk + 1] - B.spOff[chunk];
		if (G <= 2 || G > 0xFFF0u || nUniq + 1 > 0x1Fu) return;
		const DevNode* nodes = W.nodes + nBase;
		const CandStatic* packs = W.packs + W.packBase[chunk];
		const CandStatic* unkPacks = reinterpret_cast<const CandStatic*>(M.unkPacks);
		PosRec* recs = W.posRecs + W.packBase[chunk];
		const uint32_t recCap = W.packBase[chunk + 1] - W.packBase[chunk];
		uint32_t* prev = W.posPrev + nBase; uint32_t* nodeRec = W.posNodeRec + nBase;
		const uint8_t* cls = B.cls + B.charOff[chunk];

		uint32_t recTop = 0, posTop = 0;
		for (uint32_t base = 1; base + 1 < G; base += 64)
		{
			const uint32_t i = base + lane;
			const bool act = i + 1 < G;
			uint32_t cnt = 0; bool slow = false, isFirst = false;
			if (act)
			{
				const DevNode nd = nodes[i];
				if (nd.form != NOFORM)
				{
					const bool spaceBefore = nd.nflags & NF_SPACE_BEFORE;
					for (uint32_t k = 0; k < nd.candCnt; ++k)
					{
						const uint4 m1 = reinterpret_cast<const uint4*>(packs + nd.packOff + k)[1];
						const uint32_t kind = posCandKind(P, m1.y & 0xFFFF, (uint8_t)m1.z, spaceBefore);
						if (kind) ++cnt;
					}
					if (!cnt) slow = true;
					if (nd.nflags & NF_ALL_PARTIAL) ++cnt;
				}
				else cnt = 2;
				isFirst = i == 1 || nodes[i - 1].endPos != nd.endPos || nodes[i - 1].pad != nd.pad;
				const uint32_t firstPrev = i - nd.prev;
				prev[i] = firstPrev;
				uint32_t j0 = i;
				while (j0 > 1 && nodes[j0 - 1].endPos == nd.endPos && nodes[j0 - 1].pad == nd.pad) --j0;
				if (firstPrev + nd.nPrev > j0) slow = true;
			}
			uint32_t incl = cnt;
			for (uint32_t d = 1; d < 64; d <<= 1) { const uint32_t v = __shfl_up(incl, d); if (lane >= d) incl += v; }
			const uint64_t fb = __ballot(isFirst);
// ... 209 lines not shown
```

### kiwi_amd/csrc/lattice_wave.hip

```cpp
#include <hip/hip_runtime.h>
#include "device_types.hpp"
#include "feature.hpp"
#include "lattice_expand.hpp"

namespace kamd
{
	extern __shared__ __align__(16) uint8_t lSmem[];

	namespace lw
	{
		enum OpFlag : uint16_t
		{
			OF_HASUNK = 1, OF_CONDBU = 2,
			OF_LIMJ = 4, OF_HASAPP = 8, OF_SEOK = 16, OF_QUAL = 32, OF_ZBITS = 64 | 128, OF_VALID = 256, OF_ZSEL = 512 | 1024, OF_END = 2048,
		};
		constexpr uint32_t kMaxRounds = 16;

		__device__ __forceinline__ uint32_t topBit(uint64_t m) { return 63u - (uint32_t)__builtin_clzll(m); }
		__device__ __forceinline__ uint32_t trimmedLen(const uint16_t* str, uint32_t off, uint32_t len)
		{
			while (len && isSpace(str[off + len - 1])) --len;
			return len;
		}
	}

#ifdef LW_PROFILE
#define LW_T0() unsigned long long lwT = clock64(); uint32_t lwAcc[13] = {};
#define LW_MARK(k) { const unsigned long long lwN = clock64(); lwAcc[(k)] += (uint32_t)(lwN - lwT); lwT = lwN; if ((k) == 12 && lane == 0 && W.beacon) for (int lwI = 0; lwI < 13; ++lwI) W.beacon[16 * (size_t)chunk + lwI] = lwAcc[lwI]; }
#else
#define LW_T0()
#define LW_MARK(k)
#endif
#define LW_HAND_OVER(reason) { if (lane == 0) { const bool toWide = !wide && ((reason) == 0 || (reason) == 1 || (reason) == 6); W.nNodes[chunk] = toWide ? kLatticeNeedsWide : kLatticeNeedsBig; \
		if (toWide) W.wideList[atomicAdd(&W.outCounters[3], 1u)] = chunk; atomicAdd(&W.outCounters[(reason) == 6 ? 4 : 4 + (reason)], 1u); } return; }
	__global__ void __launch_bounds__(64) k_lattice_wave(ModelView M, BatchView B, WorkView W, SearchParams P, const uint32_t* chunkList, uint32_t chunkCount, uint32_t ldsBytes, uint32_t matchRatio16, uint32_t expandMode)
	{
		using namespace lw;
		const uint32_t lane = threadIdx.x;
		const bool wide = (matchRatio16 & kLatticeWideBit) != 0;
		if (wide) chunkCount = W.outCounters[3] < chunkCount ? W.outCounters[3] : chunkCount;
		if (blockIdx.x >= chunkCount) return;
		LW_T0()
		const uint32_t chunk = wide ? W.wideList[blockIdx.x] : chunkList[blockIdx.x];
		if (W.results[chunk].status >= 16) return;
		const uint32_t dbgStop = ldsBytes >> 24; ldsBytes &= 0xFFFFFFu;
#define LW_STOP(k) if (dbgStop == (k)) { if (lane == 0) W.results[chunk].status = CS_NO_LATTICE; return; }
		const uint32_t cOff = B.charOff[chunk], n = B.charOff[chunk + 1] - cOff;
		const uint32_t nNs = W.nNs[chunk];
		const uint32_t nBase = W.nodeBase[chunk], cap = W.nodeBase[chunk + 1] - nBase;
		const uint32_t mBase = W.matchBase[chunk], mCap = W.matchBase[chunk + 1] - mBase;
		if (wide && W.nNodes[chunk] != kLatticeNeedsWide) return;
		const LwLds lay = latticeWaveLayout(n, cap, mCap, matchRatio16);
		if (lay.total > ldsBytes) { if (wide && lane == 0) W.nNodes[chunk] = kLatticeNeedsBig; return; }
		if (nNs > 0xFFF0 || cap > 0xFFF0 || cap < 4) { if (lane == 0) W.results[chunk].status = CS_ERR_TOO_LONG; return; }
		uint8_t* const lS = lSmem;

		uint16_t* str = reinterpret_cast<uint16_t*>(lS + lay.str);
		uint8_t* cls = lS + lay.cls; uint8_t* script = lS + lay.script; uint8_t* cflag = lS + lay.cflag;
		uint16_t* nsToPos = reinterpret_cast<uint16_t*>(lS + lay.nsToPos); uint16_t* posToNs = reinterpret_cast<uint16_t*>(lS + lay.posToNs);
		uint64_t* mask = reinterpret_cast<uint64_t*>(lS + lay.mask); uint32_t* moff = reinterpret_cast<uint32_t*>(lS + lay.moff);
		uint32_t* mforms = reinterpret_cast<uint32_t*>(lS + lay.mforms); uint8_t* mse = lS + lay.mse; uint32_t* mfc = reinterpret_cast<uint32_t*>(lS + lay.mfc);
		uint32_t* ctlBU = reinterpret_cast<uint32_t*>(lS + lay.ctlBU); uint16_t* ctlT = reinterpret_cast<uint16_t*>(lS + lay.ctlT); uint16_t* ctlRs = reinterpret_cast<uint16_t*>(lS + lay.ctlRs);
		uint32_t* opNE = reinterpret_cast<uint32_t*>(lS + lay.opNE); uint32_t* opBU = reinterpret_cast<uint32_t*>(lS + lay.opBU);
		uint16_t* opFl = reinterpret_cast<uint16_t*>(lS + lay.opFl); uint16_t* opSrc = reinterpret_cast<uint16_t*>(lS + lay.opSrc);
		uint16_t* decS = reinterpret_cast<uint16_t*>(lS + lay.decS); uint32_t* decT = reinterpret_cast<uint32_t*>(lS + lay.decT);
		uint16_t* grpList = reinterpret_cast<uint16_t*>(lS + lay.grpList);
		uint32_t* miscForm = reinterpret_cast<uint32_t*>(lS + lay.miscForm); uint32_t* miscU = reinterpret_cast<uint32_t*>(lS + lay.miscU); uint32_t* miscFc = reinterpret_cast<uint32_t*>(lS + lay.miscFc);
		uint32_t* grpOff = reinterpret_cast<uint32_t*>(lS + lay.grpOff); uint32_t* posA = reinterpret_cast<uint32_t*>(lS + lay.posA); uint32_t* posZ = reinterpret_cast<uint32_t*>(lS + lay.posZ);
		uint64_t* fd = reinterpret_cast<uint64_t*>(lS + lay.fd); uint32_t* fdw = reinterpret_cast<uint32_t*>(lS + lay.fd);
		uint16_t* unkMinT = reinterpret_cast<uint16_t*>(lS + lay.unkMinT); uint16_t* cntU = reinterpret_cast<uint16_t*>(lS + lay.cntU); uint32_t* cntA = reinterpret_cast<uint32_t*>(lS + lay.cntA);
		uint64_t* succ = reinterpret_cast<uint64_t*>(lS + lay.succ); uint32_t* succw = reinterpret_cast<uint32_t*>(lS + lay.succ);
		uint16_t* base = reinterpret_cast<uint16_t*>(lS + lay.base); uint32_t* firstU = reinterpret_cast<uint32_t*>(lS + lay.firstU);
		uint32_t* cc = reinterpret_cast<uint32_t*>(lS + lay.cc); uint32_t* recOff = reinterpret_cast<uint32_t*>(lS + lay.recOff); uint32_t* scal = reinterpret_cast<uint32_t*>(lS + lay.scal);
		const uint32_t nPosAll = nNs + 2;

		uint32_t mTot;
		{
			const uint16_t* gstr = B.chars + cOff; const uint8_t* gcls = B.cls + cOff; const uint8_t* gscript = B.script + cOff; const uint8_t* gcflag = W.cflag + cOff;
			const uint16_t* gn2p = W.nsToPos + cOff + chunk; const uint16_t* gp2n = W.posToNs + cOff + chunk;
			const uint64_t* gmask = W.matchMask + cOff + chunk; const uint32_t* gmoff = W.matchOff + cOff + chunk;
			for (uint32_t i = lane; i < n; i += 64) { str[i] = gstr[i]; cls[i] = gcls[i]; script[i] = gscript[i]; cflag[i] = gcflag[i]; }
			for (uint32_t i = lane; i <= n; i += 64) { posToNs[i] = gp2n[i]; if (i < nNs) nsToPos[i] = gn2p[i]; }
			for (uint32_t i = lane; i <= nNs; i += 64) { mask[i] = gmask[i]; moff[i] = gmoff[i]; }
			for (uint32_t i = lane; i < nPosAll; i += 64) { ctlT[i] = 0; ctlRs[i] = 0; ctlBU[i] = 0; unkMinT[i] = 0xFFFF; cntU[i] = 0; grpOff[i] = 0; posZ[i] = 0; base[i] = 0xFFFF; }
			if (lane == 0) { grpOff[nPosAll] = 0; scal[0] = 0; scal[1] = 0; }
			mTot = gmoff[nNs] + __popcll(gmask[nNs]);
			const uint32_t* gforms = W.matchForm + mBase;
			if (mTot > lay.matchCap) LW_HAND_OVER(0)
			waveSync();
			uint16_t* endOf = grpList; uint16_t* gapPre = decS;
			for (uint32_t e = lane; e <= nNs; e += 64) { const uint32_t m0 = moff[e], c = (uint32_t)__popcll(mask[e]); for (uint32_t i = 0; i < c; ++i) endOf[m0 + i] = (uint16_t)e; }
			uint32_t run = 0;
			for (uint32_t b0 = 0; b0 < nNs; b0 += 64)
			{
				const uint32_t i = b0 + lane;
				const uint32_t g = (i > 0 && i < nNs && nsToPos[i] - nsToPos[i - 1] > 1) ? 1u : 0u;
				uint32_t incl = g;
				for (uint32_t d = 1; d < 64; d <<= 1) { const uint32_t v = __shfl_up(incl, d); if (lane >= d) incl += v; }
				if (i < nNs) gapPre[i] = (uint16_t)(run + incl);
				run += __shfl(incl, 63);
			}
		}
		waveSync();
		LW_MARK(0)
		LW_STOP(1)

		bool plain = B.patOff[chunk] == B.patOff[chunk + 1];
		for (uint32_t b0 = 0; b0 < n; b0 += 64)
		{
			const uint32_t j = b0 + lane;
			bool odd = false;
			if (j < n) { const uint16_t c = str[j]; odd = isHighSurrogate(c) || isLowSurrogate(c) || c == 0x200d || script[j] == 98; }
			if (__ballot(odd)) plain = false;
		}
		if (plain)
		{
			uint32_t tC = T_UNKNOWN, sC = 0, ssC = 0, bC = 0, uC = 0, Tbase = 1, miscBase = 0;
			bool over = false;
			auto lastEvent = [&](uint64_t ev, uint32_t val, uint32_t carry) -> uint32_t
			{
				const uint64_t m = ev & (((1ull << lane) - 1ull) | (1ull << lane));
				const uint32_t got = __shfl(val, m ? (int)topBit(m) : (int)lane);
				return m ? got : carry;
			};
			for (uint32_t b0 = 0; b0 < n; b0 += 64)
			{
				const uint32_t j = b0 + lane; const bool act = j < n;
				const uint32_t t = act ? (uint32_t)(cls[j] & 0x3F) : (uint32_t)T_UNKNOWN, sc = act ? (uint32_t)script[j] : 0u;
				const uint32_t tUp = __shfl_up(t, 1), sUp = __shfl_up(sc, 1);
				const uint32_t tp = lane ? tUp : tC, sp = lane ? sUp : sC;
				const bool symL = tp == T_SL || tp == T_SH || tp == T_SW, symC = t == T_SL || t == T_SH || t == T_SW;
				const bool disc = act && (((symL && symC) ? (sp != sc) : (tp != t)) || tp == T_SSO || tp == T_SSC);
				const bool spec = disc && tp != T_MAX && tp != T_UNKNOWN && tp != T_SS;
				const bool sjp = T_SF <= tp && tp <= T_SW;
				const bool isM = act && !disc && t == T_MAX, isS = act && t == T_UNKNOWN;
				const uint32_t pj = act ? (uint32_t)posToNs[j] : 0u, pj1 = act ? (uint32_t)posToNs[j + 1] : 0u;
				const uint32_t ss = lastEvent(__ballot(disc || isS), isS ? pj1 : pj, ssC);
				const uint32_t ssUp = __shfl_up(ss, 1); const uint32_t ssPrev = lane ? ssUp : ssC;
				const uint32_t bb = lastEvent(__ballot(isS || (disc && sjp)), isS ? pj1 : pj, bC);
				const uint32_t bUp = __shfl_up(bb, 1); const uint32_t bPrev = lane ? bUp : bC;
				const uint32_t uu = lastEvent(__ballot(isS || disc || isM), isS ? pj1 : ssPrev, uC);
				const uint32_t uUp = __shfl_up(uu, 1); const uint32_t uPrev = lane ? uUp : uC;
				uint32_t zsel = 0, zform = 0, zfl = 0;
				const bool flush = act && !isS;
				if (flush && pj < nNs)
				{
					const uint16_t ch = str[j];
					if ((P.match & M_Z_CODA) && isHangulCoda(ch) && (j + 1 >= n || !isHangulSyllable(str[j + 1]))) { zsel = 1; zform = kDefaultTagSize + (ch - 0x11A8) - 1; }
					else if ((P.match & (M_SPLIT_SAISIOT | M_MERGE_SAISIOT)) && ch == 0x11BA && j + 1 < n && isHangulSyllable(str[j + 1])) { zsel = 2; zform = kDefaultTagSize + (0x11BA - 0x11A8) - 1; }
					if (zsel)
					{
						const FormRec f = M.forms[zform];
						const uint32_t flen = f.len - f.numSpaces;
						if (flen > pj1) zsel = 0;
						else if (flen != 1) { over = true; zsel = 0; }
						else
						{
							const bool hj = (f.flags & FF_HAS_JCLASS) || (f.flags & FF_IS_STAG);
							zfl = OF_HASAPP | OF_SEOK | OF_VALID | (zsel << 9) | ((uint32_t)(f.flags & 3) << 6);
							if (!(f.flags & FF_FIRST_IS_CODA)) zfl |= OF_HASUNK | (hj ? OF_LIMJ : 0);
							if (f.flags & FF_HAS_ANY_FULL) zfl |= OF_QUAL;
						}
					}
				}
				const uint32_t nMiscMine = (spec ? 1u : 0u) + (isS ? 1u : 0u) + (zsel ? 1u : 0u);
				const uint32_t nOpsMine = nMiscMine + (flush ? (uint32_t)__popcll(mask[pj1]) : 0u);
				uint32_t inclT = nOpsMine, inclM = nMiscMine;
				for (uint32_t d = 1; d < 64; d <<= 1) { const uint32_t v = __shfl_up(inclT, d), w = __shfl_up(inclM, d); if (lane >= d) { inclT += v; inclM += w; } }
				uint32_t T = Tbase + inclT - nOpsMine, mi = miscBase + inclM - nMiscMine;
				const uint32_t totT = __shfl(inclT, 63), totM = __shfl(inclM, 63);
				if (Tbase + totT >= lay.opCap || miscBase + totM >= lay.miscCap) over = true;
				if (!over)
				{
					auto put = [&](uint32_t nb, uint32_t e, uint32_t bnd, uint32_t unk, uint32_t fl, uint32_t form, uint32_t uOff, uint32_t uLen)
					{
						opNE[T] = nb | (e << 16); opBU[T] = bnd | (unk << 16); opFl[T] = (uint16_t)fl; opSrc[T] = (uint16_t)(0x8000u | mi);
						miscForm[mi] = form; miscU[mi] = uOff | (uLen << 16);
						++T; ++mi;
					};
					if (spec)
					{
						const uint32_t o = nsToPos[ssPrev], l = trimmedLen(str, o, j - o);
						put(ssPrev, pj, bPrev, uPrev, OF_HASUNK | OF_CONDBU | (sjp ? OF_LIMJ : 0) | OF_HASAPP | OF_SEOK | OF_VALID, tp - 1u, o, l);
					}
					if (isS) put(pj1, pj1, (disc && sjp) ? pj : bPrev, (disc || isM) ? ssPrev : uPrev, OF_HASUNK | OF_CONDBU | OF_LIMJ | OF_VALID, NOFORM, 0, 0);
					if (flush)
					{
						if (zsel) put(pj1 - 1, pj1, bb, uu, zfl, zform, 0, 0);
						ctlBU[pj1] = bb | (uu << 16); ctlT[pj1] = (uint16_t)T; ctlRs[pj1] = 0;
					}
				}
				Tbase += totT; miscBase += totM;
				tC = __shfl(t, 63); sC = __shfl(sc, 63); ssC = __shfl(ss, 63); bC = __shfl(bb, 63); uC = __shfl(uu, 63);
				if (b0 + 64 > n) { const uint32_t last = (n - 1) & 63u; tC = __shfl(t, last); sC = __shfl(sc, last); }
			}
			over = __ballot(over) != 0;
			if (lane == 0)
			{
				uint32_t T = Tbase, mi = miscBase, boundary = bC, unkStart = uC; const uint32_t specialStart = ssC, lastType = tC;
				auto put = [&](uint32_t nb, uint32_t e, uint32_t fl, uint32_t form, uint32_t uOff, uint32_t uLen)
				{
					if (T >= lay.opCap || mi >= lay.miscCap) { over = true; return; }
					opNE[T] = nb | (e << 16); opBU[T] = boundary | (unkStart << 16); opFl[T] = (uint16_t)fl; opSrc[T] = (uint16_t)(0x8000u | mi);
					miscForm[mi] = form; miscU[mi] = uOff | (uLen << 16);
					++T; ++mi;
				};
				if (lastType != T_MAX && lastType != T_UNKNOWN && lastType != T_SS)
				{
					const bool sj = T_SF <= lastType && lastType <= T_SW;
					const uint32_t o = nsToPos[specialStart], l = trimmedLen(str, o, n - o);
					put(specialStart, posToNs[n], OF_HASUNK | OF_CONDBU | (sj ? OF_LIMJ : 0) | OF_HASAPP | OF_SEOK | OF_VALID, lastType - 1u, o, l);
					unkStart = specialStart;
					if (sj) boundary = posToNs[n];
				}
				if (nNs && n == (uint32_t)nsToPos[nNs - 1] + 1) put(posToNs[n], posToNs[n], OF_HASUNK | OF_CONDBU | OF_LIMJ | OF_VALID, NOFORM, 0, 0);
				put(nNs, nNs + 1, OF_HASAPP | OF_SEOK | OF_VALID | OF_END, NOFORM, 0, 0);
				scal[0] = over ? 1u : 0u; scal[1] = T - 1;
			}
		}
		else if (lane == 0)
		{
			const DevPattern* pat = B.patterns + B.patOff[chunk];
			const DevPattern* patEnd = B.patterns + B.patOff[chunk + 1];
			uint8_t lastType = T_UNKNOWN, lastScript = 0;
			uint32_t specialStart = 0, unkStart = 0, boundary = 0, resetNs = 0;
			uint32_t T = 1, nMisc = 0; bool over = false;
			const uint8_t scriptVS = 98;
			auto emit = [&](uint32_t nb, uint32_t e, uint32_t fl, uint32_t form, uint32_t uOff, uint32_t uLen)
			{
				if (T >= lay.opCap || nMisc >= lay.miscCap) { over = true; return; }
				opNE[T] = nb | (e << 16); opBU[T] = boundary | (unkStart << 16); opFl[T] = (uint16_t)fl; opSrc[T] = (uint16_t)(0x8000u | nMisc);
				miscForm[nMisc] = form; miscU[nMisc] = uOff | (uLen << 16);
				++nMisc; ++T;
			};
			for (uint32_t j = 0; j < n; ++j)
			{
				const uint16_t ch = str[j];
				const bool pair = isHighSurrogate(ch) && j + 1 < n;
				const uint32_t c32 = pair ? mergeSurrogate(ch, str[j + 1]) : ch;
				const bool inPattern = pat != patEnd && j >= pat->end - pat->length;
				uint8_t type = cls[j] & 0x3F, sct = script[j];
				bool overridden = false;
				if (lastType == T_SW && (c32 == 0x200d || (0x1f3fb <= c32 && c32 <= 0x1f3ff) || sct == scriptVS)) { overridden = type == T_UNKNOWN; type = lastType; sct = lastScript; }
				const uint8_t curT = inPattern ? (uint8_t)T_UNKNOWN : type;
				const bool symL = lastType == T_SL || lastType == T_SH || lastType == T_SW;
				const bool symC = curT == T_SL || curT == T_SH || curT == T_SW;
// ... 81 lines not shown
		uint32_t hazardEarly = 0;
		{
			const uint32_t* gforms = W.matchForm + mBase;
			const uint16_t* endOf = grpList; const uint16_t* gapPre = decS;
			for (uint32_t k = lane; k < mTot; k += 64)
			{
				const uint32_t fi = gforms[k]; const FormRec f = M.forms[fi];
				const uint32_t e = endOf[k], flen = f.len - f.numSpaces;
				const uint32_t T = (uint32_t)ctlT[e] + (k - moff[e]);
				uint32_t nb = 0, se = 0; bool valid = false;
				if (flen <= e)
				{
					valid = true; nb = e - flen;
					if (!f.numSpaces) { if (flen > 1) se = (uint32_t)gapPre[e - 1] - (uint32_t)gapPre[nb]; }
					else
					{
						const uint16_t* fs = M.formChars + f.charOff;
						uint32_t off = 0;
						for (uint32_t i = 1; i < flen; ++i)
						{
							const bool hasSpace = nsToPos[nb + i] - nsToPos[nb + i - 1] > 1;
							const uint16_t fc = (i + off < f.len) ? fs[i + off] : 0;
							if (hasSpace && fc != u' ') ++se;
							if (fc == u' ') ++off;
						}
					}
				}
				const uint8_t fl = f.flags;
				const bool hj = (fl & FF_HAS_JCLASS) || (fl & FF_IS_STAG);
				uint32_t of = OF_HASAPP | ((uint32_t)(fl & 3) << 6);
				if (!(fl & FF_FIRST_IS_CODA)) of |= OF_HASUNK | (hj ? OF_LIMJ : 0);
				if (se <= P.spaceTol) of |= OF_SEOK;
				if (fl & FF_HAS_ANY_FULL) of |= OF_QUAL;
				if (valid && nb >= ctlRs[e]) of |= OF_VALID;
				opNE[T] = nb | (e << 16); opBU[T] = ctlBU[e]; opFl[T] = (uint16_t)of; opSrc[T] = (uint16_t)k;
				mforms[k] = fi; mse[k] = (uint8_t)(se > 255 ? 255 : se);
				mfc[k] = (uint32_t)(f.candCnt & 0x7FFFu) | ((f.flags2 & FF2_ALL_PARTIAL) ? 0x8000u : 0u) | ((uint32_t)f.flags << 16) | ((uint32_t)f.len << 24);
				if (f.candCnt > 0x7FFFu) hazardEarly = 1;
				if ((of & OF_VALID) && (of & OF_SEOK) && (fl & 3)) atomicOr(&posZ[e], (uint32_t)(fl & 3));
			}
		}
		waveSync();

		if (__ballot(hazardEarly != 0)) LW_HAND_OVER(0)
		LW_MARK(2)
		for (uint32_t T = 1 + lane; T <= K; T += 64) atomicAdd(&grpOff[(opNE[T] & 0xFFFF) + 1], 1u);
		waveSync();
		{
			uint32_t run = 0;
			for (uint32_t b0 = 0; b0 <= nPosAll; b0 += 64)
			{
				const uint32_t q = b0 + lane;
				const uint32_t c = q <= nPosAll ? grpOff[q] : 0u;
				uint32_t incl = c;
				for (uint32_t d = 1; d < 64; d <<= 1) { const uint32_t v = __shfl_up(incl, d); if (lane >= d) incl += v; }
				if (q <= nPosAll) grpOff[q] = run + incl;
				if (q < nPosAll) posA[q] = 0;
				run += __shfl(incl, 63);
			}
		}
		waveSync();
		for (uint32_t T = 1 + lane; T <= K; T += 64)
		{
			const uint32_t q = opNE[T] & 0xFFFF;
			grpList[grpOff[q] + atomicAdd(&posA[q], 1u)] = (uint16_t)T;
			const uint32_t fl0 = opFl[T], zs0 = (fl0 >> 9) & 3u;
			decS[T] = (uint16_t)((1u << 4) | (((fl0 & OF_VALID) && (!zs0 || (posZ[q] & zs0))) ? (1u << 5) : 0u));
			decT[T] = 0xFFFFu << 16;
		}
		waveSync();
		for (uint32_t q = lane; q < nPosAll; q += 64)
		{
			const uint32_t g0 = grpOff[q], g1 = grpOff[q + 1];
			for (uint32_t i = g0 + 1; i < g1; ++i)
			{
				const uint16_t v = grpList[i]; uint32_t j = i;
				while (j > g0 && grpList[j - 1] > v) { grpList[j] = grpList[j - 1]; --j; }
				grpList[j] = v;
			}
		}
		waveSync();

		LW_MARK(3)
		LW_STOP(3)
		auto reachAt = [&](uint32_t x, uint32_t T) -> bool { return posA[x] < T || (uint32_t)unkMinT[x] < T; };
		uint32_t hazard = 0, nRounds = 0;
		for (uint32_t round = 0;; ++round)
		{
			if (round >= kMaxRounds) { hazard = 1; break; }
			nRounds = round + 1;
			bool chg = false;
			for (uint32_t q = lane; q < nPosAll; q += 64) { posA[q] = q ? 0xFFFFFFFFu : 0u; posZ[q] = 0; fd[q] = 0; }
			waveSync();
			LW_MARK(4)
			{
				uint32_t carry = 0;
				for (uint32_t b0 = 1; b0 <= K; b0 += 64)
				{
					const uint32_t T = b0 + lane; const bool act = T <= K;
					uint32_t fl = 0, nb = 0, e = 0, s = 0;
					if (act) { fl = opFl[T]; const uint32_t ne = opNE[T]; nb = ne & 0xFFFF; e = ne >> 16; s = decS[T]; }
					const bool app = act && (fl & OF_HASAPP) && (fl & OF_SEOK) && ((s >> 5) & 1) && ((s >> 4) & 1);
					const bool any = app || (s & 15u);
					const uint32_t lastAfter = app ? e : nb;
					const uint64_t m = __ballot(any);
					const uint64_t lower = m & ((1ull << lane) - 1ull);
					const uint32_t got = __shfl(lastAfter, lower ? (int)topBit(lower) : (int)lane);
					const uint32_t lb = lower ? got : carry;
					const uint32_t top = __shfl(lastAfter, m ? (int)topBit(m) : 0);
					if (m) carry = top;
					if (act)
					{
						const uint32_t nd = (app ? 1u : 0u) | (lb << 16);
						decT[T] = nd;
						if (app)
						{
							atomicMin(&posA[e], T);
							const uint32_t len = e - nb;
							if ((fl & OF_QUAL) && len >= 1 && len <= 64) atomicOr(&fdw[2 * e + ((len - 1) >> 5)], 1u << ((len - 1) & 31));
							const uint32_t zb = (fl >> 6) & 3u;
							if (zb) atomicOr(&posZ[e], zb);
						}
					}
				}
			}
			waveSync();
			LW_MARK(5)
			{
				uint32_t carryQ = 0xFFFFFFFFu, carryCnt = 0; uint64_t carryF = 0;
				for (uint32_t b0 = 0; b0 < K; b0 += 64)
				{
					const uint32_t g = b0 + lane; const bool act = g < K;
					uint32_t T = 0, fl = 0, q = 0xFFFFFFFEu, b = 0, u = 0, lastB = 0xFFFF, prev = 0;
					if (act) { T = grpList[g]; fl = opFl[T]; const uint32_t bu = opBU[T]; b = bu & 0xFFFF; u = bu >> 16; q = opNE[T] & 0xFFFF; lastB = decT[T] >> 16; prev = decS[T]; }
					uint64_t Fdict = 0; uint32_t rmT = 0xFFFFFFFFu, zq = 0;
					if (act) { Fdict = fd[q]; rmT = posA[q]; zq = posZ[q]; }
					bool valid = (fl & OF_VALID) != 0;
					const uint32_t zsel = (fl >> 9) & 3u;
					if (zsel) valid = valid && (zq & zsel);
					const bool tries = act && valid && (fl & OF_HASUNK);
					const uint32_t lim = (fl & OF_LIMJ) ? P.maxUnkJ : P.maxUnk;
					const bool doB = (fl & OF_CONDBU) ? (b < u) : (b < q);
					auto lenKeyOf = [&](uint32_t s0) -> uint32_t { const uint32_t o = nsToPos[s0], len = nsToPos[q - 1] + 1u - o; return plain ? len : trimmedLen(str, o, len); };
					uint32_t lp = lastB;
					if (tries && lastB < q && lp && isHangulCoda(str[nsToPos[lp]])) --lp;
					uint64_t contrib = 0;
					if (tries)
					{
						for (uint32_t a = doB ? 0u : 1u; a < 2; ++a)
						{
							const uint32_t s0 = a ? u : b;
							if (s0 >= q) continue;
							const uint32_t L = q - s0;
							if (L > 64) { hazard = 1; continue; }
							if (!((Fdict >> (L - 1)) & 1) && L <= lim && reachAt(s0, T)) { const uint32_t l = lenKeyOf(s0); if (l > 64) hazard = 1; else if (l) contrib |= 1ull << (l - 1); }
						}
						if ((prev & 5u) && lastB < q) { const uint32_t l = lenKeyOf(lp); if (l > 64) hazard = 1; else if (l) contrib |= 1ull << (l - 1); }
					}
					const uint32_t qUp = __shfl_up(q, 1);
					const bool segStart = lane == 0 ? (q != carryQ) : (q != qUp);
					const uint64_t sb = __ballot(segStart);
					const uint64_t mineSeg = sb & (((1ull << lane) - 1ull) | (1ull << lane));
					const uint32_t start = mineSeg ? topBit(mineSeg) : 0u;
					uint32_t lo = (uint32_t)contrib, hi = (uint32_t)(contrib >> 32);
					for (uint32_t d = 1; d < 64; d <<= 1)
					{
						const uint32_t vl = __shfl_up(lo, d), vh = __shfl_up(hi, d);
						if (lane >= d && lane - d >= start) { lo |= vl; hi |= vh; }
					}
					const uint32_t exLo = __shfl_up(lo, 1), exHi = __shfl_up(hi, 1);
					uint64_t F = Fdict;
					if (lane > start) F |= ((uint64_t)exHi << 32) | exLo;
					if (!mineSeg) F |= carryF;
					uint32_t um = 0, own = 0;
					if (tries)
					{
						uint32_t le = lastB;
						for (uint32_t a = doB ? 0u : 1u; a < 2; ++a)
						{
							const uint32_t s0 = a ? u : b;
							if (s0 >= q) continue;
							const uint32_t L = q - s0;
							if (L > 64) continue;
							if ((F >> (L - 1)) & 1) continue;
							if (le < q && lp != s0)
							{
								const uint32_t L2 = q - lp;
								if (L2 > 64) hazard = 1;
								else if (!((F >> (L2 - 1)) & 1) && reachAt(lp, T))
								{
									const uint32_t l = lenKeyOf(lp);
									if (l > 64) hazard = 1; else if (l) F |= 1ull << (l - 1);
									um |= 1u << (2 * a); ++own; le = q;
								}
							}
							if (L <= lim && reachAt(s0, T))
							{
								const uint32_t l = lenKeyOf(s0);
								if (l > 64) hazard = 1; else if (l) F |= 1ull << (l - 1);
								um |= 2u << (2 * a); ++own; le = q;
							}
						}
					}
					uint32_t incl = own;
					for (uint32_t d = 1; d < 64; d <<= 1) { const uint32_t v = __shfl_up(incl, d); if (lane >= d && lane - d >= start) incl += v; }
					uint32_t rank = incl - own;
					if (!mineSeg) rank += carryCnt;
					if (act)
					{
						if (rank > 250) hazard = 1;
						const bool rq = rmT < T || rank + own > 0;
						const uint32_t nd = um | (rq ? 16u : 0u) | (valid ? 32u : 0u) | ((rank & 0xFF) << 8);
#ifdef LW_DEBUG_ROUNDS
						if (prev != nd && round >= 1) printf("round %u q %u T %u fl %x old %x new %x lastB %u rmT %u nb|e %x\n", round, q, T, fl, prev, nd, lastB, rmT, opNE[T]);
#endif
						if (prev != nd) { chg = true; decS[T] = (uint16_t)nd; }
						if (own && rank == 0) base[q] = (uint16_t)T;
					}
					bool segEnd = act && lane < 63 && ((sb >> (lane + 1)) & 1);
					if (act && lane == 63) segEnd = g + 1 >= K || (opNE[grpList[g + 1]] & 0xFFFFu) != q;
					if (segEnd) { cntU[q] = (uint16_t)(rank + own); if (rank + own == 0) base[q] = 0xFFFF; }
					const uint64_t fullF = ((uint64_t)hi << 32) | lo;
					const uint32_t cLo = __shfl((uint32_t)fullF, 63), cHi = __shfl((uint32_t)(fullF >> 32), 63), cCnt = __shfl(rank + own, 63), cQ = __shfl(q, 63);
					const bool contSeg = sb == 0;
					carryF = (contSeg ? carryF : 0ull) | ((uint64_t)cHi << 32) | cLo;
					carryCnt = cCnt;
					carryQ = cQ;
				}
			}
			waveSync();
			LW_MARK(6)
#ifdef LW_DEBUG_ROUNDS
			for (uint32_t q = lane; q < nPosAll; q += 64) if (unkMinT[q] != base[q] && round >= 1) printf("round %u q %u unkMinT %u -> %u\n", round, q, (unsigned)unkMinT[q], (unsigned)base[q]);
#endif
			for (uint32_t q = lane; q < nPosAll; q += 64) if (unkMinT[q] != base[q]) { chg = true; unkMinT[q] = base[q]; }
			waveSync();
			LW_MARK(7)
			if (__ballot(hazard != 0)) { hazard = 1; break; }
			if (!__ballot(chg)) break;
		}
		if (__ballot(hazard != 0)) LW_HAND_OVER(2)
		if (!(decT[K] & 1u)) LW_HAND_OVER(3)
		if (lane == 0)
		{
			const uint32_t r100 = (mTot * 100u) / (n ? n : 1u);
			if (r100 > W.outCounters[13]) atomicMax(&W.outCounters[13], r100);
			if (matchRatio16 & 0x4000u) { atomicAdd(&W.outCounters[10], 1u); atomicAdd(&W.outCounters[11], nRounds); atomicMax(&W.outCounters[12], (K * 100u) / (n ? n : 1u)); atomicAdd(&W.outCounters[14], K); atomicAdd(&W.outCounters[15], n); }
		}

		LW_MARK(8)
		LW_STOP(4)
		uint64_t* pred = fd; uint32_t* predw = fdw;
		for (uint32_t i = lane; i < nPosAll; i += 64) { cntA[i] = 0; succ[i] = 0; firstU[i] = 0; pred[i] = 0; }
		waveSync();
		{
			uint32_t carryE = 0xFFFFFFFFu, carryCnt = 0;
			for (uint32_t b0 = 1; b0 <= K; b0 += 64)
			{
				const uint32_t T = b0 + lane; const bool act = T <= K;
				uint32_t nb = 0, e = 0xFFFFFFFEu; bool app = false;
				if (act) { const uint32_t ne = opNE[T]; nb = ne & 0xFFFF; e = ne >> 16; app = decT[T] & 1u; }
				const uint32_t ePrev = __shfl_up(e, 1);
				const bool segStart = lane == 0 ? (e != carryE) : (e != ePrev);
				const uint64_t sb = __ballot(segStart), am = __ballot(app);
				const uint64_t below = (1ull << lane) - 1ull;
				const uint64_t mine = sb & (below | (1ull << lane));
				const uint32_t start = mine ? topBit(mine) : 0u;
				uint32_t rank = (uint32_t)__popcll(am & below & ~((1ull << start) - 1ull));
				if (!mine) rank += carryCnt;
				if (act && app)
				{
					decT[T] = (decT[T] & 0xFFFF0001u) | (rank << 1);
					if (!(opFl[T] & OF_END))
					{
						const uint32_t len = e - nb;
						if (len < 1 || len > 64) hazard = 1; else { atomicOr(&succw[2 * nb + ((len - 1) >> 5)], 1u << ((len - 1) & 31)); atomicOr(&predw[2 * e + ((len - 1) >> 5)], 1u << ((len - 1) & 31)); }
						if (rank == 0) { const uint32_t src = opSrc[T]; firstU[e] = (src & 0x8000u) ? miscU[src & 0x7FFFu] : 0u; }
					}
					atomicAdd(&cntA[e], 1u);
				}
				const uint32_t eLast = __shfl(e, 63);
				const uint32_t startLast = sb ? topBit(sb) : 0u;
				const uint32_t inLast = (uint32_t)__popcll(am & ~((1ull << startLast) - 1ull));
				carryCnt = sb ? inLast : carryCnt + inLast;
				carryE = eLast;
			}
		}
		waveSync();
		for (uint32_t q = lane; q < nPosAll; q += 64)
		{
			const uint32_t g0 = grpOff[q], g1 = grpOff[q + 1];
			bool first = cntA[q] == 0 && q != 0;
			for (uint32_t g = g0; g < g1; ++g)
			{
				const uint32_t T = grpList[g]; const uint32_t s4 = decS[T] & 15u;
				if (!s4) continue;
				const uint32_t bu = opBU[T];
				uint32_t lp = decT[T] >> 16;
				if ((s4 & 5u) && lp && isHangulCoda(str[nsToPos[lp]])) --lp;
				for (uint32_t i = 0; i < 4; ++i)
				{
					if (!((s4 >> i) & 1)) continue;
					const uint32_t s = (i & 1) ? ((i & 2) ? (bu >> 16) : (bu & 0xFFFF)) : lp;
					const uint32_t len = q - s;
					atomicOr(&succw[2 * s + ((len - 1) >> 5)], 1u << ((len - 1) & 31)); atomicOr(&predw[2 * q + ((len - 1) >> 5)], 1u << ((len - 1) & 31));
					if (first) { const uint32_t o = nsToPos[s]; firstU[q] = o | (trimmedLen(str, o, nsToPos[q - 1] + 1u - o) << 16); first = false; }
				}
			}
		}
		waveSync();
		if (__ballot(hazard != 0)) LW_HAND_OVER(4)

		LW_MARK(9)
		LW_STOP(5)
		uint16_t* keep = unkMinT;
		{
			if (lane == 0)
			{
				uint64_t win = 0;
				keep[nNs + 1] = 1;
				for (uint32_t q = nNs + 1; q-- > 0;)
				{
					const bool k = q == nNs ? true : (succ[q] & win) != 0;
					keep[q] = k ? 1 : 0;
					win = (win << 1) | (k ? 1ull : 0ull);
				}
			}
		}
		waveSync();
		if (!keep[0]) LW_HAND_OVER(5)
		uint32_t nConn = 0;
		for (uint32_t b0 = 0; b0 < nPosAll; b0 += 64)
		{
			const uint32_t q = b0 + lane;
			uint32_t c = 0;
			if (q < nPosAll && keep[q]) c = q == 0 ? 1u : cntA[q] + cntU[q];
			uint32_t incl = c;
			for (uint32_t d = 1; d < 64; d <<= 1) { const uint32_t v = __shfl_up(incl, d); if (lane >= d) incl += v; }
			if (q < nPosAll) base[q] = (uint16_t)(nConn + incl - c);
			nConn += __shfl(incl, 63);
		}
		if (nConn + 1 >= cap) { if (lane == 0) W.results[chunk].status = CS_ERR_NODE_OVERFLOW; return; }
		if (nConn > lay.nodeCap) LW_HAND_OVER(6)
		waveSync();

		LW_MARK(10)
		LW_STOP(6)
		DevNode* fin = W.nodes + nBase;
		const uint32_t textOff = B.textOffset[chunk];
		auto factsOf = [&](uint32_t form) -> uint32_t { const FormRec f = M.forms[form]; return (uint32_t)(f.candCnt & 0x7FFFu) | ((f.flags2 & FF2_ALL_PARTIAL) ? 0x8000u : 0u) | ((uint32_t)f.flags << 16) | ((uint32_t)f.len << 24); };
		if (lane == 0) cc[0] = 0;
		for (uint32_t T = 1 + lane; T <= K; T += 64)
		{
			const uint32_t ne = opNE[T], nb = ne & 0xFFFF, e = ne >> 16, ds = decS[T], s4 = ds & 15u, dt = decT[T];
			if (s4 && keep[nb]) { uint32_t r = base[nb] + cntA[nb] + ((ds >> 8) & 0xFFu); for (uint32_t i = 0; i < 4; ++i) if ((s4 >> i) & 1) cc[r++] = 0; }
			if ((dt & 1u) && keep[e])
			{
				const uint32_t src = opSrc[T];
				uint32_t fc = 0;
				if (!(src & 0x8000u)) fc = mfc[src];
				else { const uint32_t form = miscForm[src & 0x7FFFu]; if (form != NOFORM) fc = factsOf(form); miscFc[src & 0x7FFFu] = fc; }
				cc[base[e] + ((dt >> 1) & 0x7FFFu)] = fc & 0x7FFFu;
			}
		}
		waveSync();
		LW_MARK(11)
		uint32_t packTop = 0;
		for (uint32_t b0 = 0; b0 < nConn; b0 += 64)
		{
			const uint32_t i = b0 + lane;
			const uint32_t c = i < nConn ? cc[i] : 0u;
			uint32_t incl = c;
			for (uint32_t d = 1; d < 64; d <<= 1) { const uint32_t v = __shfl_up(incl, d); if (lane >= d) incl += v; }
			if (i < nConn) cc[i] = packTop + incl - c;
			packTop += __shfl(incl, 63);
		}
		waveSync();
		if (packTop > W.packBase[chunk + 1] - W.packBase[chunk])
		{
			if (lane == 0) W.results[chunk].status = CS_ERR_NODE_OVERFLOW;
			return;
		}
		const bool doExpand = (expandMode & 1u) != 0, transposed = (expandMode & 2u) != 0;
		const uint32_t G = nConn;
		const uint32_t nUniq = B.spOff[chunk + 1] - B.spOff[chunk];
		CandStatic* packs = W.packs + W.packBase[chunk];
		const CandStatic* unkPacks = reinterpret_cast<const CandStatic*>(M.unkPacks);
		PosRec* recs = doExpand ? W.posRecs + W.packBase[chunk] : nullptr;
		PosDesc* desc = doExpand ? W.posDesc + nBase : nullptr;
		uint32_t* posSlow = grpOff; uint32_t* posPass1 = posA; uint32_t* posIdx = posZ;
		bool posOk = doExpand && G > 2 && G <= 0xFFF0u && nUniq + 1 <= 0x1Fu;
		uint32_t nPos = 0, recTop = 0;
		auto spaceBeforeOf = [&](uint32_t s0, bool isEnd) -> bool
		{
			const uint32_t startStr = isEnd ? n : (uint32_t)nsToPos[s0];
			return s0 == 0 ? (textOff + startStr > 0) : ((uint32_t)nsToPos[s0 - 1] + 1u < startStr);
		};
		if (doExpand)
		{
			if (lane == 0) { desc[0].firstNode = 0; desc[0].nNodes = 0; desc[0].flags = 0; desc[0].firstRec = 0; desc[0].nRec = 0; }
			for (uint32_t q = lane; q < nPosAll; q += 64) { posSlow[q] = 0; posPass1[q] = 0; }
			if (lane == 0) recOff[0] = 0;
			waveSync();
			for (uint32_t T = 1 + lane; T <= K; T += 64)
			{
				const uint32_t ne = opNE[T], nb = ne & 0xFFFF, e = ne >> 16, fl = opFl[T], ds = decS[T], s4 = ds & 15u, dt = decT[T];
				if (s4 && keep[nb])
				{
					uint32_t r = base[nb] + cntA[nb] + ((ds >> 8) & 0xFFu);
					for (uint32_t i = 0; i < 4; ++i) if ((s4 >> i) & 1) recOff[r++] = 2;
					const uint32_t bu = opBU[T];
					uint32_t lp = dt >> 16;
					if ((s4 & 5u) && lp && isHangulCoda(str[nsToPos[lp]])) --lp;
					for (uint32_t i = 0; i < 4; ++i)
					{
						if (!((s4 >> i) & 1)) continue;
						const uint32_t s0 = (i & 1) ? ((i & 2) ? (bu >> 16) : (bu & 0xFFFF)) : lp;
						if (s0 && cntA[s0] + cntU[s0] > 256) atomicOr(&posSlow[nb], 1u);
					}
				}
				if ((dt & 1u) && keep[e])
				{
					const uint32_t rank = (dt >> 1) & 0x7FFFu, src = opSrc[T], ni = base[e] + rank;
					if (fl & OF_END) { recOff[ni] = 0; continue; }
					uint32_t form, fc;
					if (src & 0x8000u) { form = miscForm[src & 0x7FFFu]; fc = miscFc[src & 0x7FFFu]; } else { form = mforms[src]; fc = mfc[src]; }
					if (nb && cntA[nb] + cntU[nb] > 256) atomicOr(&posSlow[e], 1u);
					if (form == NOFORM) { recOff[ni] = 2; continue; }
					const uint32_t candCnt = fc & 0x7FFFu, candOff = M.forms[form].candOff, pk = cc[ni];
					const bool spaceBefore = spaceBeforeOf(nb, false);
					uint32_t cnt = 0, classCnt[5] = { 0, 0, 0, 0, 0 };
					if (transposed)
						for (uint32_t k = 0; k < candCnt; ++k) { const MorphRec r = M.morphs[M.formCand[candOff + k]]; ++classCnt[candClassOf(r.tag, r.socket, r.flags)]; }
					uint32_t classAt[5] = { 0, classCnt[0], classCnt[0] + classCnt[1], classCnt[0] + classCnt[1] + classCnt[2], classCnt[0] + classCnt[1] + classCnt[2] + classCnt[3] };
					for (uint32_t k = 0; k < candCnt; ++k)
					{
						const CandStatic o = candStaticOf(M, M.formCand[candOff + k]);
						const uint32_t flags = o.m1.y & 0xFFFF; const uint8_t tag = (uint8_t)o.m1.z;
						const uint32_t at = transposed ? classAt[candClassOf(tag, o.m1.z >> 24, flags)]++ : k;
						packs[pk + at] = o;
						if (posCandKind(P, flags, tag, spaceBefore)) ++cnt;
					}
					if (cnt == 0) atomicOr(&posSlow[e], 1u);
					if ((fc & 0x8000u) && rank < 16) atomicOr(&posPass1[e], 1u << rank);
					recOff[ni] = cnt + ((fc & 0x8000u) ? 1u : 0u);
				}
			}
			waveSync();
			for (uint32_t b0 = 0; b0 < G; b0 += 64)
			{
				const uint32_t i = b0 + lane;
				const uint32_t c = i < G ? recOff[i] : 0u;
				uint32_t incl = c;
				for (uint32_t d = 1; d < 64; d <<= 1) { const uint32_t v = __shfl_up(incl, d); if (lane >= d) incl += v; }
				if (i < G) recOff[i] = recTop + incl - c;
				recTop += __shfl(incl, 63);
			}
			for (uint32_t b0 = 0; b0 < nPosAll; b0 += 64)
			{
				const uint32_t q = b0 + lane;
				const bool has = q >= 1 && q <= nNs && keep[q] && cntA[q] + cntU[q] > 0;
				const uint64_t hb = __ballot(has);
				if (q < nPosAll) posIdx[q] = has ? nPos + 1u + (uint32_t)__popcll(hb & ((1ull << lane) - 1ull)) : 0u;
				nPos += (uint32_t)__popcll(hb);
			}
			const uint32_t recCap = W.packBase[chunk + 1] - W.packBase[chunk];
			if (recTop > recCap || recTop >= 0x3FFFFu || nPos >= 0x1FFFu) posOk = false;
			waveSync();
			if (posOk)
			{
				uint32_t* posMask = W.posMask + nBase;
				bool overAny = false;
				for (uint32_t q = 1 + lane; q <= nNs; q += 64)
				{
					const uint32_t p = posIdx[q];
					if (!p) continue;
					const uint32_t n0 = base[q], nN = cntA[q] + cntU[q], r0 = recOff[n0], r1 = n0 + nN < G ? recOff[n0 + nN] : recTop;
					const bool slow = nN > 16 || r1 - r0 > 16 || r1 == r0 || posSlow[q] != 0;
					uint32_t st4[4] = { 0, 0, 0, 0 }, nSt = 0; bool over = nPos > 255;
					for (uint64_t m = pred[q]; m && !over; m &= m - 1)
					{
						const uint32_t len = (uint32_t)__ffsll((unsigned long long)m), sp = posIdx[q - len];
						if (nSt == 4) { over = true; break; }
						st4[nSt++] = sp;
					}
					for (uint32_t t = nSt; t < 4; ++t) st4[t] = st4[0];
					posMask[p] = over ? 0xFFFFFFFFu : (st4[0] | (st4[1] << 8) | (st4[2] << 16) | (st4[3] << 24));
					overAny = overAny || over;
					const uint32_t a = cntA[q], tot = nN < 16 ? nN : 16u;
					const uint32_t formless = a < 16 ? (((1u << tot) - 1u) & ~((1u << a) - 1u)) : 0u;
					PosDesc d;
					d.firstNode = (uint16_t)n0; d.nNodes = (uint8_t)(nN > 255 ? 255 : nN); d.flags = slow ? (uint8_t)POSF_SLOW : (uint8_t)0;
					d.firstRec = r0; d.nRec = (uint16_t)(r1 - r0 > 0xFFFF ? 0xFFFF : r1 - r0); d.pad = (uint16_t)formless; d.pad2 = posPass1[q];
					desc[p] = d;
				}
				if (__ballot(overAny) && lane == 0) desc[0].nNodes = 1;
				if (lane == 0)
				{
					PosDesc d; d.firstNode = (uint16_t)(G - 1); d.nNodes = 0; d.flags = 0; d.firstRec = recTop; d.nRec = 0; d.pad = 0; d.pad2 = 0;
					desc[nPos + 1] = d;
					desc[0].pad2 = posIdx[nNs];
				}
			}
		}
		auto emitNode = [&](uint32_t ni, uint32_t s, uint32_t t, uint32_t form, uint32_t fc, uint32_t uOff, uint32_t uLen, uint32_t se, uint32_t rankAt, bool isEnd)
		{
			DevNode nn;
			nn.form = form; nn.uformOff = (uint16_t)uOff; nn.uformLen = (uint16_t)uLen; nn.spaceErrors = (uint8_t)(se > 255 ? 255 : se);
			nn.ownFeat = 0; nn.pad = 0; nn.packOff = cc[ni];
			const bool pnBos = s == 0;
			const bool spaceBefore = spaceBeforeOf(s, isEnd);
			bool lb = pnBos || spaceBefore;
			const uint32_t pu = firstU[s];
			if (!lb && (pu >> 16))
			{
				const uint32_t lp = (pu & 0xFFFF) + (pu >> 16) - 1;
				const uint16_t c = str[lp];
				const uint8_t tag = (isLowSurrogate(c) || isHighSurrogate(c)) ? (uint8_t)T_SH : (uint8_t)(cls[lp] & 0x3F);
				if (tag == T_SSC || c == u'"' || c == u'\'') lb = false;
				else if (T_SF <= tag && tag <= T_SB) lb = true;
			}
			uint8_t nf = 0;
			if (spaceBefore) nf |= NF_SPACE_BEFORE;
			if (lb) nf |= NF_LEFT_BOUNDARY;
			if (uLen && str[uOff + uLen - 1] == u'.') nf |= NF_UFORM_ENDS_POINT;
			if (fc & 0x8000u) nf |= NF_ALL_PARTIAL;
			nn.nPrev = (uint16_t)(pnBos ? 1u : cntA[s] + cntU[s]);
			nn.candCnt = (uint16_t)(fc & 0x7FFFu); nn.fflags = (uint8_t)(fc >> 16); nn.flen = (uint8_t)(fc >> 24);
			if (uLen)
			{
				uint16_t of = featMaskFast(str + uOff, uLen) & 0x1FFF;
				const uint32_t lp = uOff + uLen - 1;
				const uint16_t c = str[lp];
				const uint8_t tag = (isLowSurrogate(c) || isHighSurrogate(c)) ? (uint8_t)T_SH : (uint8_t)(cls[lp] & 0x3F);
				if (tag == T_SSC) of |= LF_STR_SSC;
				nn.ownFeat = of;
			}
			nn.nflags = nf;
			nn.prev = (uint16_t)(ni - base[s]);
			nn.sibling = (!isEnd && rankAt + 1 < cntA[t] + cntU[t]) ? 1 : 0;
			if (isEnd) nn.startPos = nn.endPos = (uint16_t)n;
			else { nn.startPos = nsToPos[s]; nn.endPos = (uint16_t)(nsToPos[t - 1] + 1); }
			fin[ni] = nn;
			if (!posOk || isEnd) return;
			{
				const uint32_t np1 = (uint32_t)nn.nPrev - 1u, sp = posIdx[s];
				(W.posPrev + nBase)[ni] = base[s] | ((np1 > 255u ? 255u : np1) << 16) | ((sp > 255u ? 255u : sp) << 24);
			}
			const uint32_t nl = rankAt;
			if (nl >= 16) return;
			PosRec* out = recs + recOff[ni];
			float ws = 0;
			if (!nn.uformLen && nn.form != NOFORM && nn.flen && nn.spaceErrors) ws = -P.spacePenalty * (float)nn.spaceErrors;
			const float baseDiscount = ws + (-0.f * P.typoCostWeight);
			const uint8_t ownKind0 = nn.uformLen ? 1 : 0;
			auto emit = [&](const CandStatic* cs, float disc, uint8_t ownKind, uint16_t ownFeat, uint32_t extra)
			{
				const uint4* q4 = reinterpret_cast<const uint4*>(cs);
				const uint4 m0 = q4[0], m1 = q4[1], mx = q4[2];
				const uint8_t tag = (uint8_t)m1.z, special = (uint8_t)(m1.w >> 24);
				const uint32_t sbType = mx.z;
				const bool quote = special == 0 || special == 1 || special == 3 || special == 4;
				const uint32_t R = ((sbType || quote) && nUniq > 1) ? nUniq : 1u;
				PosRec r;
				r.firstWid = mx.y; r.secondWid = mx.w; r.chunkOff = m0.z; r.lastSeqId = m0.y;
				r.morph = mx.x; r.flagsFeat = m1.y; r.tagw = m1.z; r.cntw = m1.w;
				r.additional = __uint_as_float(m0.w) + disc + leftBoundaryScore(((nn.nflags & NF_LEFT_BOUNDARY) ? T_MAX : 0) + clearIrregular(tag)) * 5.f;
				const uint32_t ruleBits = ((isEClass(tag) && (nn.fflags & FF_STARTS_WITH_A)) ? 1u : 0u) | ((tag == T_SN && (nn.nflags & NF_UFORM_ENDS_POINT)) ? 2u : 0u)
					| ((M.morphDialect && M.morphDialect[r.morph]) ? 4u : 0u);
				r.nodeOwn = ni | ((uint32_t)ownFeat << 16);
				r.bits = (sbType & 0xFF) | (ruleBits << 8) | ((uint32_t)ownKind << 16) | ((uint32_t)nn.nflags << 24);
				r.rq = R | (nl << 8) | extra;
				*out++ = r;
			};
			auto sharedFirstWord = [&](const CandStatic* cl, uint32_t nc) -> uint32_t
			{
				if (!transposed) return 0u;
				uint32_t nReg = 0, ref = 0; bool one = true;
				for (uint32_t k = 0; k < nc; ++k)
				{
					const uint4* q4 = reinterpret_cast<const uint4*>(cl + k);
					const uint4 m1 = q4[1], mx = q4[2];
					const uint32_t flags = m1.y & 0xFFFF; const uint8_t tag = (uint8_t)m1.z, sock = (uint8_t)(m1.z >> 24);
					if (posCandKind(P, flags, tag, spaceBefore) != 1 || sock || (flags & MF_FIRST_WID_IS_P)) continue;
					if (!nReg) ref = mx.y; else if (mx.y != ref) one = false;
					++nReg;
				}
				return (nReg && one) ? (uint32_t)PR_OUT_FIRST : 0u;
			};
			if (nn.form != NOFORM)
			{
				const CandStatic* cl = packs + nn.packOff;
				const uint32_t of0 = sharedFirstWord(cl, nn.candCnt);
				for (uint32_t k = 0; k < nn.candCnt; ++k)
				{
					const uint4 m1 = reinterpret_cast<const uint4*>(cl + k)[1];
					const uint32_t kind = posCandKind(P, m1.y & 0xFFFF, (uint8_t)m1.z, spaceBefore);
					if (kind == 1) emit(cl + k, baseDiscount + 0.f, ownKind0, nn.ownFeat, of0);
					else if (kind == 2)
					{
						const MorphRec cm = M.morphs[reinterpret_cast<const uint4*>(cl + k)[2].x];
						const MorphRec nm = M.morphs[cm.lmId];
						PosRec r;
						r.firstWid = cm.lmId; r.secondWid = cm.tag; r.chunkOff = (uint32_t)nm.feat | ((uint32_t)nm.prevFlags << 16) | (nm.socket ? 1u << 24 : 0u); r.lastSeqId = 0;
						r.morph = cm.lmId; r.flagsFeat = 0; r.tagw = 0; r.cntw = 0;
						r.additional = cm.userScore;
						r.nodeOwn = ni; r.bits = (uint32_t)nn.nflags << 24; r.rq = 1u | (nl << 8) | (uint32_t)PR_Z;
						*out++ = r;
					}
				}
				if (nn.nflags & NF_ALL_PARTIAL)
				{
					const FormRec f = M.forms[nn.form];
					uint16_t of = featMaskFast(M.formChars + f.charOff, f.len) & 0x1FFF;
					if (f.flags & FF_ENDS_WITH_SSC) of |= LF_STR_SSC;
					const float disc = baseDiscount + -((float)f.len * P.oovRuleScale + P.oovRuleBias);
					emit(unkPacks + 1, disc, 2, of, (uint32_t)PR_PASS1 | sharedFirstWord(unkPacks + 1, 1));
				}
			}
			else
			{
				const float emo = (cls[nn.uformOff] & 0x80) ? -10.f : 0.f;
				const float disc = baseDiscount + (emo - ((float)nn.uformLen * P.oovRuleScale + P.oovRuleBias));
				const uint32_t of0 = sharedFirstWord(unkPacks, 2);
				emit(unkPacks, disc, ownKind0, nn.ownFeat, of0);
				emit(unkPacks + 1, disc, ownKind0, nn.ownFeat, of0);
			}
		};
		if (lane == 0)
		{
			DevNode bos; bos.form = NOFORM; bos.startPos = bos.endPos = 0; bos.prev = bos.sibling = 0; bos.uformOff = bos.uformLen = 0; bos.spaceErrors = 0; bos.nflags = 0; bos.nPrev = 0; bos.packOff = 0; bos.candCnt = 0; bos.fflags = 0; bos.flen = 0; bos.ownFeat = 0; bos.pad = 0;
			fin[0] = bos;
		}
		for (uint32_t T = 1 + lane; T <= K; T += 64)
		{
			const uint32_t ne = opNE[T], nb = ne & 0xFFFF, e = ne >> 16, fl = opFl[T], s4 = decS[T] & 15u, dt = decT[T];
			if (s4 && keep[nb])
			{
				const uint32_t bu = opBU[T];
				uint32_t lp = dt >> 16;
				if ((s4 & 5u) && lp && isHangulCoda(str[nsToPos[lp]])) --lp;
				uint32_t r = cntA[nb] + ((decS[T] >> 8) & 0xFFu);
				for (uint32_t i = 0; i < 4; ++i)
				{
					if (!((s4 >> i) & 1)) continue;
					const uint32_t s0 = (i & 1) ? ((i & 2) ? (bu >> 16) : (bu & 0xFFFF)) : lp;
					const uint32_t o = nsToPos[s0], len = nsToPos[nb - 1] + 1u - o, l = plain ? len : trimmedLen(str, o, len);
					emitNode(base[nb] + r, s0, nb, NOFORM, 0, o, l, 0, r, false);
					++r;
				}
			}
			if ((dt & 1u) && keep[e])
			{
				const uint32_t rank = (dt >> 1) & 0x7FFFu, src = opSrc[T];
				uint32_t form, fc, uOff = 0, uLen = 0, se = 0;
				if (src & 0x8000u) { form = miscForm[src & 0x7FFFu]; fc = miscFc[src & 0x7FFFu]; const uint32_t mu = miscU[src & 0x7FFFu]; uOff = mu & 0xFFFF; uLen = mu >> 16; }
				else { form = mforms[src]; fc = mfc[src]; se = mse[src]; }
				emitNode(base[e] + rank, nb, e, form, fc, uOff, uLen, se, rank, (fl & OF_END) != 0);
			}
		}
		if (doExpand)
		{
			waveSync();
			if (lane == 0) { if (posOk) desc[0].firstRec = nPos; W.expanded[chunk] = 1; }
		}
		LW_MARK(12)
		if (lane == 0)
		{
			const uint32_t packCap = W.packBase[chunk + 1] - W.packBase[chunk];
			if (packTop > packCap) W.results[chunk].status = CS_ERR_NODE_OVERFLOW;
			else { W.nNodes[chunk] = nConn; if (nConn <= 2) W.results[chunk].status = CS_NO_LATTICE; }
		}
	}
}
```

Measured before the change: 14.90 million sentences/s.

## Precompute per-form candidate rows at model load and use DPP wave scans

Builds a device table of per-form candidate records, already in class-transposed order, once at model load. The lattice kernel then copies these rows with vector loads instead of recounting classes and rebuilding each record per node, and emitNode reads the table directly. Shuffle-based wave prefix sums are replaced with DPP row shifts plus readlane, and a probe kernel is added to test the scans. The cost is extra device memory for the table and reliance on the precomputed order matching the per-chunk order.

```diff
diff --git a/include/kiwi_amd.h b/include/kiwi_amd.h
--- a/include/kiwi_amd.h
+++ b/include/kiwi_amd.h
@@ -56,6 +56,8 @@
 
 int kamd_debug_exact_math(const float* x, float* exp_out, float* log_out, uint32_t n);
 int kamd_debug_exact_tanh(const float* x, float* tanh_out, uint32_t n);
+int kamd_debug_wave_scan(const uint32_t* x, const uint32_t* start, const uint32_t* or_lo, const uint32_t* or_hi, uint32_t* sum_out, uint32_t* seg_sum_out, uint32_t* seg_or_lo_out, uint32_t* seg_or_hi_out,
+	uint32_t* last_out, uint32_t n_cases);
 int kamd_debug_cong_global(kamd_engine_h h, const uint32_t* ctx, const uint32_t* hist7, const uint32_t* next, const uint8_t* flags, float* out, uint32_t n);
 uint64_t kamd_debug_match_pattern(uint16_t left, const uint16_t* text, uint32_t len, uint64_t match_options);
 int kamd_debug_sbg_next(const char* raw_model_path, uint32_t* hist8, uint32_t* pos, uint32_t wid, float knlm_ll, float* ll_out);
diff --git a/kiwi_amd/csrc/capi_low.cpp b/kiwi_amd/csrc/capi_low.cpp
--- a/kiwi_amd/csrc/capi_low.cpp
+++ b/kiwi_amd/csrc/capi_low.cpp
@@ -17,6 +17,7 @@
 	"kamd_token_t is the layout of kamd::FlatToken");
 
 namespace kamd { void exactMathProbe(const float* x, float* e, float* l, float* t, uint32_t n); }
+namespace kamd { void waveScanProbe(const uint32_t* x, const uint32_t* start, const uint32_t* lo, const uint32_t* hi, uint32_t* sum, uint32_t* seg, uint32_t* orLo, uint32_t* orHi, uint32_t* last, uint32_t nCases); }
 namespace kamd { void conggProbe(const FlatModel& m, const uint32_t* ctx, const uint32_t* hist, const uint32_t* next, const uint8_t* flags, float* out, uint32_t n); }
 
 namespace
@@ -278,6 +279,12 @@
 		return guarded([&]() { kamd::exactMathProbe(x, nullptr, nullptr, tanh_out, n); return 0; }, -1);
 	}
 
+	int kamd_debug_wave_scan(const uint32_t* x, const uint32_t* start, const uint32_t* or_lo, const uint32_t* or_hi, uint32_t* sum_out, uint32_t* seg_sum_out, uint32_t* seg_or_lo_out, uint32_t* seg_or_hi_out,
+		uint32_t* last_out, uint32_t n_cases)
+	{
+		return guarded([&]() { kamd::waveScanProbe(x, start, or_lo, or_hi, sum_out, seg_sum_out, seg_or_lo_out, seg_or_hi_out, last_out, n_cases); return 0; }, -1);
+	}
+
 	int kamd_debug_cong_global(kamd_engine_h h, const uint32_t* ctx, const uint32_t* hist7, const uint32_t* next, const uint8_t* flags, float* out, uint32_t n)
 	{
 		if (!h) return -1;
diff --git a/kiwi_amd/csrc/engine.hip b/kiwi_amd/csrc/engine.hip
--- a/kiwi_amd/csrc/engine.hip
+++ b/kiwi_amd/csrc/engine.hip
@@ -25,6 +25,7 @@
 #include "typo_lattice_kernel.hpp"
 #include "typo_graph_kernel.hpp"
 #include "cong_query_kernel.hpp"
+#include "wave_scan.hpp"
 
 namespace kamd
 {
@@ -33,6 +34,7 @@
 	__global__ void k_build_lattice_big(ModelView M, BatchView B, WorkView W, SearchParams P, uint32_t chunkBegin, uint32_t chunkCount, uint32_t ldsBytes, uint32_t waveLayout);
 	__global__ void k_lattice_wave(ModelView M, BatchView B, WorkView W, SearchParams P, const uint32_t* chunkList, uint32_t chunkCount, uint32_t ldsBytes, uint32_t matchRatio16, uint32_t expandMode);
 	__global__ void k_expand_cands(ModelView M, BatchView B, WorkView W, uint32_t chunkBegin, uint32_t chunkCount, uint32_t transposedOrder, const uint8_t* distMask);
+	__global__ void k_fill_cand_rows(ModelView M, CandStatic* rows, uint32_t nForms, uint32_t nCand, uint32_t transposedOrder);
 	__global__ void k_expand_pos(ModelView M, BatchView B, WorkView W, SearchParams P, uint32_t chunkBegin, uint32_t chunkCount, const float* nodeTypoAll, uint32_t useChr);
 	__global__ void k_unk_chr(ModelView M, BatchView B, WorkView W, ChrView C, uint32_t chunkBegin, uint32_t chunkCount, uint32_t hiTok, uint32_t loTok);
 	__global__ void k_unk_chr_freq(ModelView M, BatchView B, WorkView W, ChrView C, ChrFreqParams Q, float chrBias, uint32_t chunkBegin, uint32_t chunkCount, uint32_t hiTok, uint32_t loTok);
@@ -239,6 +241,7 @@
 		int device = 0;
 		uint32_t persistBlocks = 0;
 		int latticeGroupForced = 0;
+		bool latticeExpand = true;
 		bool latticeWave = true;
 		uint32_t latticeRatio16 = kLatticeWideRatio16; bool latticeRatioForced = false;
 		uint32_t stateScale64[2] = { 0, 0 }; bool stateScaleForced = false;
@@ -373,6 +376,17 @@
 		}
 		else { v.lmHash = impl->up(m.lmHash); v.lmHashMask = m.lmHashMask; v.lmRoot2 = impl->up(m.lmRoot2); v.lmBackoff = impl->up(m.lmBackoff); }
 		v.lmHtxNode = (m.congDim || m.lmHtxNode.empty()) ? nullptr : impl->up(m.lmHtxNode);
+		{
+			impl->modelBufs.emplace_back(new DevBuf);
+			DevBuf& rows = *impl->modelBufs.back();
+			const uint32_t nForms = (uint32_t)m.forms.size(), nCand = (uint32_t)m.formCand.size();
+			rows.ensure(std::max<size_t>((size_t)nCand * sizeof(CandStatic), 16));
+			HIPCHECK(hipMemsetAsync(rows.p, 0, (size_t)nCand * sizeof(CandStatic), impl->stream));
+			if (nForms) hipLaunchKernelGGL(k_fill_cand_rows, dim3((nForms + 255) / 256), dim3(256), 0, impl->stream, v, rows.as<CandStatic>(), nForms, nCand, impl->hasCong ? 1u : 0u);
+			HIPCHECK(hipGetLastError());
+			HIPCHECK(hipStreamSynchronize(impl->stream));
+			v.candRows = rows.p;
+		}
 		v.formDialect = nullptr;
 		v.morphDialect = m.morphDialect.empty() ? nullptr : impl->up(m.morphDialect, I_::kTempMorphs);
 		if (v.morphDialect) HIPCHECK(hipMemset(const_cast<uint16_t*>(v.morphDialect) + m.morphDialect.size(), 0, 2 * I_::kTempMorphs));
@@ -421,6 +435,7 @@
 		if (const char* pc = std::getenv("KAMD_POS_CONT")) impl->posContSlots = (uint32_t)std::max(0, std::min(4096, std::atoi(pc)));
 		if (const char* lg = std::getenv("KAMD_LATTICE_GROUP")) { const int v = std::atoi(lg); if (v == 16 || v == 64) impl->latticeGroupForced = v; }
 		if (const char* lw = std::getenv("KAMD_LATTICE_WAVE")) impl->latticeWave = std::atoi(lw) != 0;
+		if (const char* le = std::getenv("KAMD_LATTICE_EXPAND")) impl->latticeExpand = std::atoi(le) != 0;
 		if (const char* ss = std::getenv("KAMD_STATE_SCALE")) { impl->stateScale64[0] = impl->stateScale64[1] = (uint32_t)std::min(64, std::max(1, std::atoi(ss))); impl->stateScaleForced = true; }
 		if (const char* ps = std::getenv("KAMD_STATE_POOL")) { impl->poolFrac64 = (uint32_t)std::min(4096, std::max(0, std::atoi(ps))); impl->poolForced = true; }
 		if (const char* lr = std::getenv("KAMD_LATTICE_RATIO")) { impl->latticeRatio16 = (uint32_t)std::min(4096, std::max(4, std::atoi(lr))); impl->latticeRatioForced = true; }
@@ -825,6 +840,33 @@
 		if (t) HIPCHECK(hipMemcpy(t, dt.p, (size_t)n * 4, hipMemcpyDeviceToHost));
 	}
 
+	__global__ void __launch_bounds__(64) k_wave_scan_probe(const uint32_t* x, const uint32_t* start, const uint32_t* lo, const uint32_t* hi, uint32_t* sum, uint32_t* seg, uint32_t* orLo, uint32_t* orHi, uint32_t* last)
+	{
+		const size_t i = (size_t)blockIdx.x * 64 + threadIdx.x;
+		const uint32_t s = waveInclSum(x[i]);
+		sum[i] = s;
+		seg[i] = waveSegInclSum(x[i], start[i]);
+		uint32_t l = lo[i], h = hi[i];
+		waveSegInclOr(l, h, start[i]);
+		orLo[i] = l; orHi[i] = h;
+		const uint32_t tot = waveLast(s);
+		if (threadIdx.x == 0) last[blockIdx.x] = tot;
+	}
+	void waveScanProbe(const uint32_t* x, const uint32_t* start, const uint32_t* lo, const uint32_t* hi, uint32_t* sum, uint32_t* seg, uint32_t* orLo, uint32_t* orHi, uint32_t* last, uint32_t nCases)
+	{
+		if (!nCases) return;
+		const size_t bytes = (size_t)nCases * 64 * 4;
+		DevBuf in[4], out[4], dLast;
+		const uint32_t* src[4] = { x, start, lo, hi }; uint32_t* dst[4] = { sum, seg, orLo, orHi };
+		for (int k = 0; k < 4; ++k) { in[k].ensure(bytes); out[k].ensure(bytes); HIPCHECK(hipMemcpy(in[k].p, src[k], bytes, hipMemcpyHostToDevice)); }
+		dLast.ensure((size_t)nCases * 4 + 16);
+		hipLaunchKernelGGL(k_wave_scan_probe, dim3(nCases), dim3(64), 0, 0, in[0].as<uint32_t>(), in[1].as<uint32_t>(), in[2].as<uint32_t>(), in[3].as<uint32_t>(),
+			out[0].as<uint32_t>(), out[1].as<uint32_t>(), out[2].as<uint32_t>(), out[3].as<uint32_t>(), dLast.as<uint32_t>());
+		HIPCHECK(hipGetLastError());
+		for (int k = 0; k < 4; ++k) HIPCHECK(hipMemcpy(dst[k], out[k].p, bytes, hipMemcpyDeviceToHost));
+		HIPCHECK(hipMemcpy(last, dLast.p, (size_t)nCases * 4, hipMemcpyDeviceToHost));
+	}
+
 	__global__ void k_congg_probe(CongView C, const uint32_t* ctx, const uint32_t* hist, const uint32_t* next, const uint8_t* flags, float* out, uint32_t n)
 	{
 		const uint32_t i = blockIdx.x * blockDim.x + threadIdx.x;
@@ -1039,7 +1081,7 @@
 			{
 				const bool wave = I.latticeWave && I.latticeGroupForced == 0;
 				const uint32_t ratio16 = I.latticeRatio16 | (getenv("KAMD_LATTICE_STATS") ? 0x4000u : 0u);
-				static const bool fuseExpand = !(getenv("KAMD_LATTICE_EXPAND") && std::atoi(getenv("KAMD_LATTICE_EXPAND")) == 0);
+				const bool fuseExpand = I.latticeExpand;
 				const bool posEarly = b.wv.posRecs && sp.topN == 1 && !I.groupLanesForced && S <= 8 && (!b.typo.typo || I.posPathTypo);
 				const uint32_t expandMode = (fuseExpand && posEarly && !b.wv.unkChr && !b.wv.blockBits) ? (1u | (I.hasCong ? 2u : 0u)) : 0u;
 				if (getenv("KAMD_LATTICE_PROFILE")) { lwProf.ensure((size_t)nC * 64); HIPCHECK(hipMemsetAsync(lwProf.p, 0, (size_t)nC * 64, sA)); b.wv.beacon = lwProf.as<uint32_t>(); }
@@ -1291,12 +1333,12 @@
 		{
 			std::vector<uint32_t> rec((size_t)nC * 16);
 			HIPCHECK(hipMemcpy(rec.data(), lwProf.p, rec.size() * 4, hipMemcpyDeviceToHost));
-			double pr[13] = {}; uint32_t seen = 0;
-			for (uint32_t c = 0; c < nC; ++c) { if (!rec[(size_t)c * 16]) continue; ++seen; for (int k2 = 0; k2 < 13; ++k2) pr[k2] += rec[(size_t)c * 16 + k2]; }
-			static const char* names[13] = { "stage", "type pass", "match ops", "groups", "clear", "by-time", "by-start", "publish", "checks", "ranks", "sweep+prefix", "emit", "pack offsets" };
-			double tot = 0; for (int k2 = 0; k2 < 13; ++k2) tot += pr[k2];
+			double pr[15] = {}; uint32_t seen = 0;
+			for (uint32_t c = 0; c < nC; ++c) { if (!rec[(size_t)c * 16]) continue; ++seen; for (int k2 = 0; k2 < 15; ++k2) pr[k2] += rec[(size_t)c * 16 + k2]; }
+			static const char* names[15] = { "stage", "type pass", "match ops", "groups", "clear", "by-time", "by-start", "publish", "checks", "ranks", "sweep+prefix", "candidate counts", "pack offsets + candidate rows", "position table", "nodes + records" };
+			double tot = 0; for (int k2 = 0; k2 < 15; ++k2) tot += pr[k2];
 			fprintf(stderr, "[lattice profile] clock ticks per wavefront (%u chunks):", seen);
-			for (int k2 = 0; k2 < 13; ++k2) fprintf(stderr, " %s %.0f (%.0f%%);", names[k2], seen ? pr[k2] / seen : 0.0, tot ? 100.0 * pr[k2] / tot : 0.0);
+			for (int k2 = 0; k2 < 15; ++k2) fprintf(stderr, " %s %.0f (%.0f%%);", names[k2], seen ? pr[k2] / seen : 0.0, tot ? 100.0 * pr[k2] / tot : 0.0);
 			fprintf(stderr, " total %.0f\n", seen ? tot / seen : 0.0);
 		}
 		if (getenv("KAMD_LATTICE_STATS"))
@@ -1308,8 +1350,8 @@
 			uint32_t nEx = 0, nProg = 0;
 			for (uint32_t c = 0; c < nC; ++c) if (ex[c]) { ++nEx; if (b.wv.posDesc) { PosDesc d; HIPCHECK(hipMemcpy(&d, b.wv.posDesc + b.nodeBase[c], sizeof(d), hipMemcpyDeviceToHost)); nProg += d.firstRec != 0; } }
 			fprintf(stderr, "[lattice wave] records written by the lattice kernel: %u chunks (%u with a position program)\n", nEx, nProg);
-			fprintf(stderr, "[lattice wave] chunks %u: built %u (%.2f rounds each); handed over: matches %u, ops %u, long span / rounds %u, no end node %u, long node %u, no start %u; ops per text unit: mean %.2f, max %.2f (matches: max %.2f)\n",
-				(uint32_t)nC, c16[10], c16[10] ? (double)c16[11] / c16[10] : 0.0, c16[4], c16[5], c16[6], c16[7], c16[8], c16[9], c16[15] ? (double)c16[14] / c16[15] : 0.0, c16[12] / 100.0, c16[13] / 100.0);
+			fprintf(stderr, "[lattice wave] chunks %u: built %u (%.2f rounds each); handed over: matches %u, ops %u, long span / rounds %u, no end node %u, long node %u, no start %u; ops per text unit: mean %.2f, max %.2f (matches: max %.2f); ops %u in %u text units\n",
+				(uint32_t)nC, c16[10], c16[10] ? (double)c16[11] / c16[10] : 0.0, c16[4], c16[5], c16[6], c16[7], c16[8], c16[9], c16[15] ? (double)c16[14] / c16[15] : 0.0, c16[12] / 100.0, c16[13] / 100.0, c16[14], c16[15]);
 		}
 		if (b.wv.posRecs && getenv("KAMD_POS_STATS"))
 		{
diff --git a/kiwi_amd/csrc/flat_model.hpp b/kiwi_amd/csrc/flat_model.hpp
--- a/kiwi_amd/csrc/flat_model.hpp
+++ b/kiwi_amd/csrc/flat_model.hpp
@@ -129,6 +129,7 @@
 		const LmRootRec* lmRoot2;
 		const LmBackoff* lmBackoff;
 		const void* unkPacks;
+		const void* candRows;
 		const int32_t* lmHtxNode;
 		const float* formUnkChr;
 		const uint16_t* formChrTok;
@@ -396,7 +397,7 @@
 			v.lmHtxNode = lmHtxNode.empty() ? nullptr : lmHtxNode.data();
 			v.formUnkChr = formUnkChr.empty() ? nullptr : formUnkChr.data();
 			v.formChrTok = formChrTok.empty() ? nullptr : formChrTok.data();
-			v.lmChain = nullptr;
+			v.lmChain = nullptr; v.unkPacks = nullptr; v.candRows = nullptr;
 			v.trieEdges = trieEdges.empty() ? nullptr : trieEdges.data(); v.trieEdgeMask = trieEdgeMask;
 			v.formDialect = formDialect.empty() ? nullptr : formDialect.data(); v.morphDialect = morphDialect.empty() ? nullptr : morphDialect.data();
 			return v;
diff --git a/kiwi_amd/csrc/lattice_kernels.hip b/kiwi_amd/csrc/lattice_kernels.hip
--- a/kiwi_amd/csrc/lattice_kernels.hip
+++ b/kiwi_amd/csrc/lattice_kernels.hip
@@ -804,6 +804,28 @@
 		}
 	}
 
+	__global__ void __launch_bounds__(256) k_fill_cand_rows(ModelView M, CandStatic* rows, uint32_t nForms, uint32_t nCand, uint32_t transposedOrder)
+	{
+		const uint32_t f = blockIdx.x * blockDim.x + threadIdx.x;
+		if (f >= nForms) return;
+		const FormRec fr = M.forms[f];
+		const uint32_t candOff = fr.candOff, candCnt = fr.candCnt;
+		if (candOff > nCand || candCnt > nCand - candOff) return;
+		uint32_t classAt[5] = { 0, 0, 0, 0, 0 };
+		if (transposedOrder)
+		{
+			uint32_t classCnt[5] = { 0, 0, 0, 0, 0 };
+			for (uint32_t k = 0; k < candCnt; ++k) { const MorphRec r = M.morphs[M.formCand[candOff + k]]; ++classCnt[candClassOf(r.tag, r.socket, r.flags)]; }
+			for (uint32_t c = 1; c < 5; ++c) classAt[c] = classAt[c - 1] + classCnt[c - 1];
+		}
+		for (uint32_t k = 0; k < candCnt; ++k)
+		{
+			const CandStatic o = candStaticOf(M, M.formCand[candOff + k]);
+			const uint32_t at = transposedOrder ? classAt[candClassOf((uint8_t)o.m1.z, o.m1.z >> 24, o.m1.y & 0xFFFF)]++ : k;
+			rows[candOff + at] = o;
+		}
+	}
+
 	__global__ void __launch_bounds__(64) k_expand_pos(ModelView M, BatchView B, WorkView W, SearchParams P, uint32_t chunkBegin, uint32_t chunkCount, const float* nodeTypoAll, uint32_t useChr)
 	{
 		if (blockIdx.x >= chunkCount) return;
diff --git a/kiwi_amd/csrc/lattice_wave.hip b/kiwi_amd/csrc/lattice_wave.hip
--- a/kiwi_amd/csrc/lattice_wave.hip
+++ b/kiwi_amd/csrc/lattice_wave.hip
@@ -2,6 +2,7 @@
 #include "device_types.hpp"
 #include "feature.hpp"
 #include "lattice_expand.hpp"
+#include "wave_scan.hpp"
 
 namespace kamd
 {
@@ -25,8 +26,8 @@
 	}
 
 #ifdef LW_PROFILE
-#define LW_T0() unsigned long long lwT = clock64(); uint32_t lwAcc[13] = {};
-#define LW_MARK(k) { const unsigned long long lwN = clock64(); lwAcc[(k)] += (uint32_t)(lwN - lwT); lwT = lwN; if ((k) == 12 && lane == 0 && W.beacon) for (int lwI = 0; lwI < 13; ++lwI) W.beacon[16 * (size_t)chunk + lwI] = lwAcc[lwI]; }
+#define LW_T0() unsigned long long lwT = clock64(); uint32_t lwAcc[15] = {};
+#define LW_MARK(k) { const unsigned long long lwN = clock64(); lwAcc[(k)] += (uint32_t)(lwN - lwT); lwT = lwN; if ((k) == 14 && lane == 0 && W.beacon) for (int lwI = 0; lwI < 15; ++lwI) W.beacon[16 * (size_t)chunk + lwI] = lwAcc[lwI]; }
 #else
 #define LW_T0()
 #define LW_MARK(k)
@@ -95,10 +96,9 @@
 			{
 				const uint32_t i = b0 + lane;
 				const uint32_t g = (i > 0 && i < nNs && nsToPos[i] - nsToPos[i - 1] > 1) ? 1u : 0u;
-				uint32_t incl = g;
-				for (uint32_t d = 1; d < 64; d <<= 1) { const uint32_t v = __shfl_up(incl, d); if (lane >= d) incl += v; }
+				const uint32_t incl = waveInclSum(g);
 				if (i < nNs) gapPre[i] = (uint16_t)(run + incl);
-				run += __shfl(incl, 63);
+				run += waveLast(incl);
 			}
 		}
 		waveSync();
@@ -165,10 +165,9 @@
 				}
 				const uint32_t nMiscMine = (spec ? 1u : 0u) + (isS ? 1u : 0u) + (zsel ? 1u : 0u);
 				const uint32_t nOpsMine = nMiscMine + (flush ? (uint32_t)__popcll(mask[pj1]) : 0u);
-				uint32_t inclT = nOpsMine, inclM = nMiscMine;
-				for (uint32_t d = 1; d < 64; d <<= 1) { const uint32_t v = __shfl_up(inclT, d), w = __shfl_up(inclM, d); if (lane >= d) { inclT += v; inclM += w; } }
+				const uint32_t inclT = waveInclSum(nOpsMine), inclM = waveInclSum(nMiscMine);
 				uint32_t T = Tbase + inclT - nOpsMine, mi = miscBase + inclM - nMiscMine;
-				const uint32_t totT = __shfl(inclT, 63), totM = __shfl(inclM, 63);
+				const uint32_t totT = waveLast(inclT), totM = waveLast(inclM);
 				if (Tbase + totT >= lay.opCap || miscBase + totM >= lay.miscCap) over = true;
 				if (!over)
 				{
@@ -191,7 +190,7 @@
 					}
 				}
 				Tbase += totT; miscBase += totM;
-				tC = __shfl(t, 63); sC = __shfl(sc, 63); ssC = __shfl(ss, 63); bC = __shfl(bb, 63); uC = __shfl(uu, 63);
+				tC = waveLast(t); sC = waveLast(sc); ssC = waveLast(ss); bC = waveLast(bb); uC = waveLast(uu);
 				if (b0 + 64 > n) { const uint32_t last = (n - 1) & 63u; tC = __shfl(t, last); sC = __shfl(sc, last); }
 			}
 			over = __ballot(over) != 0;
@@ -379,11 +378,10 @@
 			{
 				const uint32_t q = b0 + lane;
 				const uint32_t c = q <= nPosAll ? grpOff[q] : 0u;
-				uint32_t incl = c;
-				for (uint32_t d = 1; d < 64; d <<= 1) { const uint32_t v = __shfl_up(incl, d); if (lane >= d) incl += v; }
+				const uint32_t incl = waveInclSum(c);
 				if (q <= nPosAll) grpOff[q] = run + incl;
 				if (q < nPosAll) posA[q] = 0;
-				run += __shfl(incl, 63);
+				run += waveLast(incl);
 			}
 		}
 		waveSync();
@@ -490,11 +488,7 @@
 					const uint64_t mineSeg = sb & (((1ull << lane) - 1ull) | (1ull << lane));
 					const uint32_t start = mineSeg ? topBit(mineSeg) : 0u;
 					uint32_t lo = (uint32_t)contrib, hi = (uint32_t)(contrib >> 32);
-					for (uint32_t d = 1; d < 64; d <<= 1)
-					{
-						const uint32_t vl = __shfl_up(lo, d), vh = __shfl_up(hi, d);
-						if (lane >= d && lane - d >= start) { lo |= vl; hi |= vh; }
-					}
+					waveSegInclOr(lo, hi, start);
 					const uint32_t exLo = __shfl_up(lo, 1), exHi = __shfl_up(hi, 1);
 					uint64_t F = Fdict;
 					if (lane > start) F |= ((uint64_t)exHi << 32) | exLo;
@@ -529,8 +523,7 @@
 							}
 						}
 					}
-					uint32_t incl = own;
-					for (uint32_t d = 1; d < 64; d <<= 1) { const uint32_t v = __shfl_up(incl, d); if (lane >= d && lane - d >= start) incl += v; }
+					const uint32_t incl = waveSegInclSum(own, start);
 					uint32_t rank = incl - own;
 					if (!mineSeg) rank += carryCnt;
 					if (act)
@@ -548,7 +541,7 @@
 					if (act && lane == 63) segEnd = g + 1 >= K || (opNE[grpList[g + 1]] & 0xFFFFu) != q;
 					if (segEnd) { cntU[q] = (uint16_t)(rank + own); if (rank + own == 0) base[q] = 0xFFFF; }
 					const uint64_t fullF = ((uint64_t)hi << 32) | lo;
-					const uint32_t cLo = __shfl((uint32_t)fullF, 63), cHi = __shfl((uint32_t)(fullF >> 32), 63), cCnt = __shfl(rank + own, 63), cQ = __shfl(q, 63);
+					const uint32_t cLo = waveLast((uint32_t)fullF), cHi = waveLast((uint32_t)(fullF >> 32)), cCnt = waveLast(rank + own), cQ = waveLast(q);
 					const bool contSeg = sb == 0;
 					carryF = (contSeg ? carryF : 0ull) | ((uint64_t)cHi << 32) | cLo;
 					carryCnt = cCnt;
@@ -606,7 +599,7 @@
 					}
 					atomicAdd(&cntA[e], 1u);
 				}
-				const uint32_t eLast = __shfl(e, 63);
+				const uint32_t eLast = waveLast(e);
 				const uint32_t startLast = sb ? topBit(sb) : 0u;
 				const uint32_t inLast = (uint32_t)__popcll(am & ~((1ull << startLast) - 1ull));
 				carryCnt = sb ? inLast : carryCnt + inLast;
@@ -662,10 +655,9 @@
 			const uint32_t q = b0 + lane;
 			uint32_t c = 0;
 			if (q < nPosAll && keep[q]) c = q == 0 ? 1u : cntA[q] + cntU[q];
-			uint32_t incl = c;
-			for (uint32_t d = 1; d < 64; d <<= 1) { const uint32_t v = __shfl_up(incl, d); if (lane >= d) incl += v; }
+			const uint32_t incl = waveInclSum(c);
 			if (q < nPosAll) base[q] = (uint16_t)(nConn + incl - c);
-			nConn += __shfl(incl, 63);
+			nConn += waveLast(incl);
 		}
 		if (nConn + 1 >= cap) { if (lane == 0) W.results[chunk].status = CS_ERR_NODE_OVERFLOW; return; }
 		if (nConn > lay.nodeCap) LW_HAND_OVER(6)
@@ -697,10 +689,9 @@
 		{
 			const uint32_t i = b0 + lane;
 			const uint32_t c = i < nConn ? cc[i] : 0u;
-			uint32_t incl = c;
-			for (uint32_t d = 1; d < 64; d <<= 1) { const uint32_t v = __shfl_up(incl, d); if (lane >= d) incl += v; }
+			const uint32_t incl = waveInclSum(c);
 			if (i < nConn) cc[i] = packTop + incl - c;
-			packTop += __shfl(incl, 63);
+			packTop += waveLast(incl);
 		}
 		waveSync();
 		if (packTop > W.packBase[chunk + 1] - W.packBase[chunk])
@@ -713,6 +704,7 @@
 		const uint32_t nUniq = B.spOff[chunk + 1] - B.spOff[chunk];
 		CandStatic* packs = W.packs + W.packBase[chunk];
 		const CandStatic* unkPacks = reinterpret_cast<const CandStatic*>(M.unkPacks);
+		const CandStatic* candRows = reinterpret_cast<const CandStatic*>(M.candRows);
 		PosRec* recs = doExpand ? W.posRecs + W.packBase[chunk] : nullptr;
 		PosDesc* desc = doExpand ? W.posDesc + nBase : nullptr;
 		uint32_t* posSlow = grpOff; uint32_t* posPass1 = posA; uint32_t* posIdx = posZ;
@@ -756,17 +748,13 @@
 					if (form == NOFORM) { recOff[ni] = 2; continue; }
 					const uint32_t candCnt = fc & 0x7FFFu, candOff = M.forms[form].candOff, pk = cc[ni];
 					const bool spaceBefore = spaceBeforeOf(nb, false);
-					uint32_t cnt = 0, classCnt[5] = { 0, 0, 0, 0, 0 };
-					if (transposed)
-						for (uint32_t k = 0; k < candCnt; ++k) { const MorphRec r = M.morphs[M.formCand[candOff + k]]; ++classCnt[candClassOf(r.tag, r.socket, r.flags)]; }
-					uint32_t classAt[5] = { 0, classCnt[0], classCnt[0] + classCnt[1], classCnt[0] + classCnt[1] + classCnt[2], classCnt[0] + classCnt[1] + classCnt[2] + classCnt[3] };
+					const uint4* rows = reinterpret_cast<const uint4*>(candRows + candOff); uint4* dst = reinterpret_cast<uint4*>(packs + pk);
+					uint32_t cnt = 0;
 					for (uint32_t k = 0; k < candCnt; ++k)
 					{
-						const CandStatic o = candStaticOf(M, M.formCand[candOff + k]);
-						const uint32_t flags = o.m1.y & 0xFFFF; const uint8_t tag = (uint8_t)o.m1.z;
-						const uint32_t at = transposed ? classAt[candClassOf(tag, o.m1.z >> 24, flags)]++ : k;
-						packs[pk + at] = o;
-						if (posCandKind(P, flags, tag, spaceBefore)) ++cnt;
+						const uint4 r0 = rows[3 * k], r1 = rows[3 * k + 1], r2 = rows[3 * k + 2];
+						dst[3 * k] = r0; dst[3 * k + 1] = r1; dst[3 * k + 2] = r2;
+						if (posCandKind(P, r1.y & 0xFFFF, (uint8_t)r1.z, spaceBefore)) ++cnt;
 					}
 					if (cnt == 0) atomicOr(&posSlow[e], 1u);
 					if ((fc & 0x8000u) && rank < 16) atomicOr(&posPass1[e], 1u << rank);
@@ -774,14 +762,14 @@
 				}
 			}
 			waveSync();
+			LW_MARK(12)
 			for (uint32_t b0 = 0; b0 < G; b0 += 64)
 			{
 				const uint32_t i = b0 + lane;
 				const uint32_t c = i < G ? recOff[i] : 0u;
-				uint32_t incl = c;
-				for (uint32_t d = 1; d < 64; d <<= 1) { const uint32_t v = __shfl_up(incl, d); if (lane >= d) incl += v; }
+				const uint32_t incl = waveInclSum(c);
 				if (i < G) recOff[i] = recTop + incl - c;
-				recTop += __shfl(incl, 63);
+				recTop += waveLast(incl);
 			}
 			for (uint32_t b0 = 0; b0 < nPosAll; b0 += 64)
 			{
@@ -830,6 +818,7 @@
 				}
 			}
 		}
+		LW_MARK(13)
 		auto emitNode = [&](uint32_t ni, uint32_t s, uint32_t t, uint32_t form, uint32_t fc, uint32_t uOff, uint32_t uLen, uint32_t se, uint32_t rankAt, bool isEnd)
 		{
 			DevNode nn;
@@ -917,7 +906,7 @@
 			};
 			if (nn.form != NOFORM)
 			{
-				const CandStatic* cl = packs + nn.packOff;
+				const CandStatic* cl = candRows + M.forms[form].candOff;
 				const uint32_t of0 = sharedFirstWord(cl, nn.candCnt);
 				for (uint32_t k = 0; k < nn.candCnt; ++k)
 				{
@@ -991,7 +980,7 @@
 			waveSync();
 			if (lane == 0) { if (posOk) desc[0].firstRec = nPos; W.expanded[chunk] = 1; }
 		}
-		LW_MARK(12)
+		LW_MARK(14)
 		if (lane == 0)
 		{
 			const uint32_t packCap = W.packBase[chunk + 1] - W.packBase[chunk];
diff --git a/kiwi_amd/csrc/wave_scan.hpp b/kiwi_amd/csrc/wave_scan.hpp
--- /dev/null
+++ b/kiwi_amd/csrc/wave_scan.hpp
@@ -0,0 +1,78 @@
+#pragma once
+#include <hip/hip_runtime.h>
+#include <cstdint>
+
+namespace kamd
+{
+#ifdef KAMD_HIPEMU
+	__device__ __forceinline__ uint32_t waveLast(uint32_t x) { return __shfl(x, 63); }
+	__device__ __forceinline__ uint32_t waveInclSum(uint32_t x)
+	{
+		const uint32_t lane = threadIdx.x & 63u;
+		for (uint32_t d = 1; d < 64; d <<= 1) { const uint32_t v = __shfl_up(x, d); if (lane >= d) x += v; }
+		return x;
+	}
+	__device__ __forceinline__ uint32_t waveSegInclSum(uint32_t x, uint32_t start)
+	{
+		const uint32_t lane = threadIdx.x & 63u;
+		for (uint32_t d = 1; d < 64; d <<= 1) { const uint32_t v = __shfl_up(x, d); if (lane >= d && lane - d >= start) x += v; }
+		return x;
+	}
+	__device__ __forceinline__ void waveSegInclOr(uint32_t& lo, uint32_t& hi, uint32_t start)
+	{
+		const uint32_t lane = threadIdx.x & 63u;
+		for (uint32_t d = 1; d < 64; d <<= 1)
+		{
+			const uint32_t vl = __shfl_up(lo, d), vh = __shfl_up(hi, d);
+			if (lane >= d && lane - d >= start) { lo |= vl; hi |= vh; }
+		}
+	}
+#else
+	namespace wsdetail
+	{
+		template<int D> __device__ __forceinline__ uint32_t rowShr(uint32_t x) { return (uint32_t)__builtin_amdgcn_update_dpp(0, (int)x, 0x110 + D, 0xF, 0xF, false); }
+		__device__ __forceinline__ uint32_t rowEnd(uint32_t x, int lane) { return (uint32_t)__builtin_amdgcn_readlane((int)x, lane); }
+	}
+	__device__ __forceinline__ uint32_t waveLast(uint32_t x) { return wsdetail::rowEnd(x, 63); }
+	__device__ __forceinline__ uint32_t waveInclSum(uint32_t x)
+	{
+		using namespace wsdetail;
+		const uint32_t lane = threadIdx.x & 63u;
+		x += rowShr<1>(x); x += rowShr<2>(x); x += rowShr<4>(x); x += rowShr<8>(x);
+		x += (lane >= 16 && lane < 32) ? rowEnd(x, 15) : 0u;
+		x += (lane >= 32 && lane < 48) ? rowEnd(x, 31) : 0u;
+		x += lane >= 48 ? rowEnd(x, 47) : 0u;
+		return x;
+	}
+	__device__ __forceinline__ uint32_t waveSegInclSum(uint32_t x, uint32_t start)
+	{
+		using namespace wsdetail;
+		const uint32_t lane = threadIdx.x & 63u;
+		const uint32_t room = lane - start;
+		uint32_t v;
+		v = rowShr<1>(x); x += room >= 1 ? v : 0u;
+		v = rowShr<2>(x); x += room >= 2 ? v : 0u;
+		v = rowShr<4>(x); x += room >= 4 ? v : 0u;
+		v = rowShr<8>(x); x += room >= 8 ? v : 0u;
+		x += (lane >= 16 && lane < 32 && start < 16) ? rowEnd(x, 15) : 0u;
+		x += (lane >= 32 && lane < 48 && start < 32) ? rowEnd(x, 31) : 0u;
+		x += (lane >= 48 && start < 48) ? rowEnd(x, 47) : 0u;
+		return x;
+	}
+	__device__ __forceinline__ void waveSegInclOr(uint32_t& lo, uint32_t& hi, uint32_t start)
+	{
+		using namespace wsdetail;
+		const uint32_t lane = threadIdx.x & 63u;
+		const uint32_t room = lane - start;
+		uint32_t vl, vh;
+		vl = rowShr<1>(lo); vh = rowShr<1>(hi); if (room >= 1) { lo |= vl; hi |= vh; }
+		vl = rowShr<2>(lo); vh = rowShr<2>(hi); if (room >= 2) { lo |= vl; hi |= vh; }
+		vl = rowShr<4>(lo); vh = rowShr<4>(hi); if (room >= 4) { lo |= vl; hi |= vh; }
+		vl = rowShr<8>(lo); vh = rowShr<8>(hi); if (room >= 8) { lo |= vl; hi |= vh; }
+		uint32_t cl, ch;
+		cl = rowEnd(lo, 15); ch = rowEnd(hi, 15); if (lane >= 16 && lane < 32 && start < 16) { lo |= cl; hi |= ch; }
+		cl = rowEnd(lo, 31); ch = rowEnd(hi, 31); if (lane >= 32 && lane < 48 && start < 32) { lo |= cl; hi |= ch; }
+		cl = rowEnd(lo, 47); ch = rowEnd(hi, 47); if (lane >= 48 && start < 48) { lo |= cl; hi |= ch; }
+	}
+#endif
+}
```

Measured after the change: 15.06 million sentences/s, median of 6. 1.01x the previous value.
